# Zhengjun-Du/LC-CRF-SLAM

Hardware: NVIDIA B200
Metric: crf_problems_per_s (higher is better)
Workload: dtype f32

## Files before the change

### include/lccrf.h

```cpp
#ifndef LCCRF_H
#define LCCRF_H

#include <stdint.h>

#ifdef __cplusplus
extern "C" {
#endif

#define LCCRF_OK 0
#define LCCRF_ERR_ARG (-1)
#define LCCRF_ERR_CUDA (-2)
#define LCCRF_ERR_STATE (-3)
#define LCCRF_ERR_RANGE (-4)

#define LCCRF_MAX_D 7
#define LCCRF_MAX_L 64
#define LCCRF_MAX_K 8

typedef struct lccrf_ctx lccrf_ctx;
typedef struct lccrf_lattice lccrf_lattice;
typedef struct lccrf_crf lccrf_crf;
typedef struct lccrf_frames lccrf_frames;

const char *lccrf_version(void);
const char *lccrf_last_error(void);
int lccrf_device_count(void);
int lccrf_ctx_create(int device, lccrf_ctx **out);
void lccrf_ctx_destroy(lccrf_ctx *ctx);
int lccrf_ctx_set_stream(lccrf_ctx *ctx, void *cuda_stream);
int lccrf_ctx_sync(lccrf_ctx *ctx);
uint64_t lccrf_ctx_kernel_launches(const lccrf_ctx *ctx);
int lccrf_ctx_build_scratch_in_use(lccrf_ctx *ctx, long long *slots);
int lccrf_ctx_set_option(lccrf_ctx *ctx, const char *name, int value);
int lccrf_ctx_profile_report(lccrf_ctx *ctx, char *buf, int cap);

int lccrf_lattice_create(lccrf_ctx *ctx, const float *features, int d, int N, lccrf_lattice **out);
void lccrf_lattice_destroy(lccrf_lattice *lat);
int lccrf_lattice_sizes(const lccrf_lattice *lat, int *N, int *d, int *V);
int lccrf_lattice_export(const lccrf_lattice *lat, int *offset, float *bary, int *nbr);
int lccrf_lattice_filter(lccrf_lattice *lat, float *out, const float *in, int L);
int lccrf_lattice_filter_window(lccrf_lattice *lat, float *out, const float *in, int L, int in_offset, int out_offset,
                                int in_size, int out_size);

int lccrf_crf_create(lccrf_ctx *ctx, int N, int L, lccrf_crf **out);
void lccrf_crf_destroy(lccrf_crf *crf);
int lccrf_crf_set_unary(lccrf_crf *crf, const float *unary);
int lccrf_crf_set_unary_from_label(lccrf_crf *crf, const short *label, float u_energy,
                                   const float *n_energies, const float *p_energies);
int lccrf_crf_set_unary_entry(lccrf_crf *crf, int idx, int m, float value);
int lccrf_crf_add_potts(lccrf_crf *crf, const float *features, int d, float w);
int lccrf_crf_add_potts_image(lccrf_crf *crf, int W, int H, float w, float posdev, const void *img,
                              int img_is_u8, int F, float featuredev);
int lccrf_crf_start(lccrf_crf *crf);
int lccrf_crf_step(lccrf_crf *crf, float relax);
int lccrf_crf_inference(lccrf_crf *crf, int n_iterations, int with_map, float relax);
int lccrf_crf_build_map(lccrf_crf *crf);
const short *lccrf_crf_map(lccrf_crf *crf);
const float *lccrf_crf_prob(lccrf_crf *crf);
int lccrf_crf_potts_vertices(const lccrf_crf *crf, int k, int *V);
int lccrf_crf_num_potts(const lccrf_crf *crf);

int lccrf_crf_potts_apply(lccrf_crf *crf, int k, float *out, const float *in, float *tmp);
int lccrf_crf_step_init(lccrf_crf *crf, float *next);
int lccrf_crf_set_prob(lccrf_crf *crf, const float *prob);
int lccrf_exp_and_normalize(lccrf_ctx *ctx, float *out, const float *in, int N, int L, float scale,
                            float relax);

typedef struct lccrf_slam_params {
    float w1, w2;
    float u_alpha, stdev_alpha;
    float u_beta, stdev_beta;
    float u_gamma, stdev_gamma;
    float point3d_stdev, point2d_stdev;
    float u_depth, pth, confidence;
    int iters;
} lccrf_slam_params;

int lccrf_map_point_unary(lccrf_ctx *ctx, int N, const float *xyz, const int *obs_ptr, const int *obs_kf,
                          const float *obs_uv, int nKF, const float *kf_pose, const float *kf_intr,
                          const float *kf_bounds, float *observs, float *error, float *depth);
int lccrf_rough_classify(lccrf_ctx *ctx, int N, const float *observs, const float *error, const float *depth,
                         const double *p4, const lccrf_slam_params *prm, short *label);

int lccrf_epipolar_prior(lccrf_ctx *ctx, int M, const int *fid1, const float *pt1, const float *pt2,
                         const double *F9, float u_gamma, float stdev_gamma, int nFeat, double *dis_by_fid,
                         double *prob_by_fid, double *dis, double *prob);
int lccrf_bf_match(lccrf_ctx *ctx, int nq, const uint8_t *desc_q, int nt, const uint8_t *desc_t, double ratio,
                   int *match, int *knn, int *n_match);
int lccrf_bf_match_batch(lccrf_ctx *ctx, int B, const int *q_ptr, const uint8_t *desc_q, const int *t_ptr,
                         const uint8_t *desc_t, double ratio, int *match, int *knn, int *n_match);

int lccrf_frames_create(lccrf_ctx *ctx, int B, const int *prob_ptr, const lccrf_slam_params *prm,
                        const float *energies3, lccrf_frames **out);
void lccrf_frames_destroy(lccrf_frames *fr);
int lccrf_frames_set_inputs(lccrf_frames *fr, const float *observs, const float *error, const float *depth,
                            const float *kp2d);
int lccrf_frames_set_map_inputs(lccrf_frames *fr, const float *xyz, const int *obs_ptr, const int *obs_kf,
                                const float *obs_uv, int nKF, const float *kf_pose, const float *kf_intr,
                                const float *kf_bounds, const float *kp2d, const int *kf_ptr);
int lccrf_frames_run(lccrf_frames *fr);
int lccrf_frames_get_outputs(lccrf_frames *fr, short *map, float *prob);
int lccrf_frames_submit_map(lccrf_frames *fr, int slot, const float *xyz, const int *obs_ptr, const void *obs_kf,
                            int obs_kf_bytes, const float *obs_uv, int nKF, const float *kf_pose, const float *kf_intr,
                            const float *kf_bounds, const float *kp2d, const int *kf_ptr, short *map_out,
                            float *prob_out);
int lccrf_frames_set_keyframe_keypoints(lccrf_frames *fr, int kf_first, int kf_count, int stride, const float *kp_uv);
int lccrf_frames_set_map_inputs_indexed(lccrf_frames *fr, const float *xyz, const int *obs_ptr, const void *obs_ref,
                                        int index_bytes, int nKF, const float *kf_pose, const float *kf_intr,
                                        const float *kf_bounds, const float *kp2d, const int *kf_ptr);
int lccrf_frames_submit_map_indexed(lccrf_frames *fr, int slot, const float *xyz, const int *obs_ptr, const void *obs_ref,
                                    int index_bytes, int nKF, const float *kf_pose, const float *kf_intr,
                                    const float *kf_bounds, const float *kp2d, const int *kf_ptr, short *map_out,
                                    float *prob_out);
int lccrf_frames_submit(lccrf_frames *fr, int slot, const float *observs, const float *error, const float *depth,
                        const float *kp2d, short *map_out, float *prob_out);
int lccrf_frames_wait(lccrf_frames *fr, int slot);
int lccrf_frames_partition(lccrf_frames *fr, const int *fid, int *dyn_ptr, int *dyn_list, int *stat_ptr,
                           int *stat_list);
int lccrf_frames_get_debug(lccrf_frames *fr, short *init_label, float *observs, float *error, float *depth,
                           int *V);
int lccrf_frames_debug_counters(lccrf_frames *fr, int k, int *out8);
int lccrf_frames_algorithmic_bytes(lccrf_frames *fr, double *total, double *per_iteration, double *unary);

typedef struct lccrf_images lccrf_images;
typedef struct lccrf_image_kernel {
    int F;
    float w, posdev, featuredev;
} lccrf_image_kernel;
int  lccrf_images_create(lccrf_ctx *ctx, int B, const int *W, const int *H, int C, int L, int K,
                         const lccrf_image_kernel *kernels, lccrf_images **out);
void lccrf_images_destroy(lccrf_images *im);
int  lccrf_images_set_inputs(lccrf_images *im, const void *img, int img_is_u8, const float *unary);
int  lccrf_images_set_inputs_from_label(lccrf_images *im, const void *img, int img_is_u8, const short *label,
                                        float u_energy, const float *n_energies, const float *p_energies);
int  lccrf_images_run(lccrf_images *im, int n_iterations, float relax);
int  lccrf_images_get_outputs(lccrf_images *im, short *map, float *prob);
int  lccrf_images_vertices(lccrf_images *im, int *V);

typedef struct lccrf_map lccrf_map;
typedef struct lccrf_map_delta {
    int kf_first, kf_count;
    const float *kf_pose, *kf_intr, *kf_bounds, *kf_keypoints;
    int n_pose;
    const int *pose_kf;
    const float *pose;
    int n_xyz;
    const int *xyz_id;
    const float *xyz;
    int n_erase;
    const int *erase_pt, *erase_kf;
    int n_bad;
    const int *bad_pt;
    int n_add;
    const int *add_pt, *add_kf, *add_fid;
    int n_erase_seg;
    const int *erase_seg_ptr;
    int n_add_seg;
    const int *add_seg_ptr;
} lccrf_map_delta;
int lccrf_map_create(lccrf_ctx *ctx, int kp_stride, lccrf_map **out);
void lccrf_map_destroy(lccrf_map *map);
int lccrf_map_apply(lccrf_map *map, const lccrf_map_delta *delta);
int lccrf_map_set_observations(lccrf_map *map, int pt_first, int count, const int *obs_ptr, const int *obs_ref);
int lccrf_map_reserve_observations(lccrf_map *map, long long entries);
int lccrf_map_sizes(lccrf_map *map, int *n_kf, int *n_points, long long *n_obs, long long *pool_used, long long *pool_cap);
int lccrf_map_export(lccrf_map *map, int n, const int *point_id, int *obs_ptr, int *obs_kf, float *obs_uv, long long cap,
                     float *xyz);

int lccrf_frames_set_visible(lccrf_frames *fr, lccrf_map *map, const lccrf_map_delta *delta, const int *point_id,
                             const float *kp2d, const int *kf_ptr);
int lccrf_frames_submit_visible(lccrf_frames *fr, int slot, lccrf_map *map, const lccrf_map_delta *delta,
                                const int *point_id, const float *kp2d, const int *kf_ptr, short *map_out, float *prob_out);
int lccrf_frames_set_prior(lccrf_frames *fr, int slot, const double *p4, const unsigned char *has_prior);
int lccrf_frames_set_partition_outputs(lccrf_frames *fr, int slot, const int *fid, int *dyn_ptr, int *dyn_list, int *stat_ptr,
                                       int *stat_list);

typedef struct lccrf_snapshot_writer lccrf_snapshot_writer;
typedef struct lccrf_snapshot_reader lccrf_snapshot_reader;
typedef struct lccrf_snapshot_info {
    int N, nKF;
    long long nnz;
    long long frame_id;
    double timestamp;
    int stored_kf_bytes;
} lccrf_snapshot_info;
int lccrf_snapshot_writer_open(const char *path, int append, lccrf_snapshot_writer **out);
int lccrf_snapshot_write_frame(lccrf_snapshot_writer *w, long long frame_id, double timestamp, int N, const float *xyz,
                               const int *obs_ptr, const int *obs_kf, const float *obs_uv, int nKF, const float *kf_pose,
                               const float *kf_intr, const float *kf_bounds, const float *kp2d, const int *fid);
int lccrf_snapshot_writer_close(lccrf_snapshot_writer *w);
int lccrf_snapshot_reader_open(const char *path, lccrf_snapshot_reader **out);
void lccrf_snapshot_reader_close(lccrf_snapshot_reader *r);
int lccrf_snapshot_num_frames(const lccrf_snapshot_reader *r);
int lccrf_snapshot_truncated(const lccrf_snapshot_reader *r);
int lccrf_snapshot_frame_info(const lccrf_snapshot_reader *r, int i, lccrf_snapshot_info *info);
int lccrf_snapshot_read_frame(lccrf_snapshot_reader *r, int i, float *xyz, int *obs_ptr, void *obs_kf, int obs_kf_bytes,
                              float *obs_uv, float *kf_pose, float *kf_intr, float *kf_bounds, float *kp2d, int *fid);

#ifdef __cplusplus
}
#endif
#endif
```

### lc-crf-slam_b200/__init__.py

```python
from __future__ import annotations

import ctypes as C
import os
import subprocess
import weakref

import numpy as np

HERE = os.path.dirname(os.path.abspath(__file__))
LIB_PATH = os.path.join(HERE, "liblccrf.so")
INCLUDE_DIR = os.path.join(os.path.dirname(HERE), "include")
DENSECRF_INCLUDE_DIR = os.path.join(HERE, "densecrf")

from . import synth


def build(verbose: bool = False) -> str:
    subprocess.run(["make", "-C", os.path.join(HERE, "csrc"), "-j8"], check=True,
                   stdout=None if verbose else subprocess.DEVNULL)
    return LIB_PATH


class LccrfError(RuntimeError):
    pass


class SlamParams(C.Structure):
    _fields_ = [(n, C.c_float) for n in (
        "w1", "w2", "u_alpha", "stdev_alpha", "u_beta", "stdev_beta", "u_gamma", "stdev_gamma",
        "point3d_stdev", "point2d_stdev", "u_depth", "pth", "confidence")] + [("iters", C.c_int)]

    @classmethod
    def make(cls, **kw) -> "SlamParams":
        p = cls()
        d = dict(synth.SLAM_PARAMS)
        d.update(kw)
        for k, v in d.items():
            setattr(p, k, v)
        return p


class ImageKernel(C.Structure):
    _fields_ = [("F", C.c_int), ("w", C.c_float), ("posdev", C.c_float), ("featuredev", C.c_float)]


_fp = C.POINTER(C.c_float)
_ip = C.POINTER(C.c_int)
_sp = C.POINTER(C.c_short)
_vp = C.c_void_p
_byref = C.byref

SYMBOLS = {
    "lccrf_version": (C.c_char_p, []),
    "lccrf_last_error": (C.c_char_p, []),
    "lccrf_device_count": (C.c_int, []),
    "lccrf_ctx_create": (C.c_int, [C.c_int, C.POINTER(_vp)]),
    "lccrf_ctx_destroy": (None, [_vp]),
    "lccrf_ctx_set_stream": (C.c_int, [_vp, _vp]),
    "lccrf_ctx_sync": (C.c_int, [_vp]),
    "lccrf_ctx_kernel_launches": (C.c_uint64, [_vp]),
    "lccrf_ctx_build_scratch_in_use": (C.c_int, [_vp, _vp]),
    "lccrf_ctx_set_option": (C.c_int, [_vp, C.c_char_p, C.c_int]),
    "lccrf_ctx_profile_report": (C.c_int, [_vp, C.c_char_p, C.c_int]),
    "lccrf_lattice_create": (C.c_int, [_vp, _vp, C.c_int, C.c_int, C.POINTER(_vp)]),
    "lccrf_lattice_destroy": (None, [_vp]),
    "lccrf_lattice_sizes": (C.c_int, [_vp, _ip, _ip, _ip]),
    "lccrf_lattice_export": (C.c_int, [_vp, _vp, _vp, _vp]),
    "lccrf_lattice_filter": (C.c_int, [_vp, _vp, _vp, C.c_int]),
    "lccrf_lattice_filter_window": (C.c_int, [_vp, _vp, _vp, C.c_int, C.c_int, C.c_int, C.c_int, C.c_int]),
    "lccrf_crf_create": (C.c_int, [_vp, C.c_int, C.c_int, C.POINTER(_vp)]),
    "lccrf_crf_destroy": (None, [_vp]),
    "lccrf_crf_set_unary": (C.c_int, [_vp, _vp]),
    "lccrf_crf_set_unary_from_label": (C.c_int, [_vp, _vp, C.c_float, _vp, _vp]),
    "lccrf_crf_set_unary_entry": (C.c_int, [_vp, C.c_int, C.c_int, C.c_float]),
    "lccrf_crf_add_potts": (C.c_int, [_vp, _vp, C.c_int, C.c_float]),
    "lccrf_crf_add_potts_image": (C.c_int, [_vp, C.c_int, C.c_int, C.c_float, C.c_float, _vp, C.c_int, C.c_int, C.c_float]),
    "lccrf_crf_start": (C.c_int, [_vp]),
    "lccrf_crf_step": (C.c_int, [_vp, C.c_float]),
    "lccrf_crf_inference": (C.c_int, [_vp, C.c_int, C.c_int, C.c_float]),
    "lccrf_crf_build_map": (C.c_int, [_vp]),
    "lccrf_crf_map": (_sp, [_vp]),
    "lccrf_crf_prob": (_fp, [_vp]),
    "lccrf_crf_potts_vertices": (C.c_int, [_vp, C.c_int, _ip]),
    "lccrf_crf_num_potts": (C.c_int, [_vp]),
    "lccrf_crf_step_init": (C.c_int, [_vp, _vp]),
    "lccrf_crf_set_prob": (C.c_int, [_vp, _vp]),
    "lccrf_crf_potts_apply": (C.c_int, [_vp, C.c_int, _vp, _vp, _vp]),
    "lccrf_exp_and_normalize": (C.c_int, [_vp, _vp, _vp, C.c_int, C.c_int, C.c_float, C.c_float]),
    "lccrf_map_point_unary": (C.c_int, [_vp, C.c_int, _vp, _vp, _vp, _vp, C.c_int, _vp, _vp, _vp, _vp, _vp, _vp]),
    "lccrf_rough_classify": (C.c_int, [_vp, C.c_int, _vp, _vp, _vp, _vp, C.POINTER(SlamParams), _vp]),
    "lccrf_epipolar_prior": (C.c_int, [_vp, C.c_int, _vp, _vp, _vp, _vp, C.c_float, C.c_float, C.c_int, _vp, _vp, _vp, _vp]),
    "lccrf_bf_match": (C.c_int, [_vp, C.c_int, _vp, C.c_int, _vp, C.c_double, _vp, _vp, _ip]),
    "lccrf_bf_match_batch": (C.c_int, [_vp, C.c_int, _vp, _vp, _vp, _vp, C.c_double, _vp, _vp, _ip]),
    "lccrf_frames_create": (C.c_int, [_vp, C.c_int, _vp, C.POINTER(SlamParams), _vp, C.POINTER(_vp)]),
    "lccrf_frames_destroy": (None, [_vp]),
    "lccrf_frames_set_inputs": (C.c_int, [_vp, _vp, _vp, _vp, _vp]),
    "lccrf_frames_set_map_inputs": (C.c_int, [_vp, _vp, _vp, _vp, _vp, C.c_int, _vp, _vp, _vp, _vp, _vp]),
    "lccrf_frames_run": (C.c_int, [_vp]),
    "lccrf_frames_get_outputs": (C.c_int, [_vp, _vp, _vp]),
    "lccrf_frames_submit_map": (C.c_int, [_vp, C.c_int, _vp, _vp, _vp, C.c_int, _vp, C.c_int, _vp, _vp, _vp, _vp, _vp, _vp, _vp]),
    "lccrf_frames_set_keyframe_keypoints": (C.c_int, [_vp, C.c_int, C.c_int, C.c_int, _vp]),
    "lccrf_frames_set_map_inputs_indexed": (C.c_int, [_vp, _vp, _vp, _vp, C.c_int, C.c_int, _vp, _vp, _vp, _vp, _vp]),
    "lccrf_frames_submit_map_indexed": (C.c_int, [_vp, C.c_int, _vp, _vp, _vp, C.c_int, C.c_int, _vp, _vp, _vp, _vp, _vp, _vp, _vp]),
    "lccrf_frames_submit": (C.c_int, [_vp, C.c_int, _vp, _vp, _vp, _vp, _vp, _vp]),
    "lccrf_frames_wait": (C.c_int, [_vp, C.c_int]),
    "lccrf_frames_partition": (C.c_int, [_vp, _vp, _vp, _vp, _vp, _vp]),
    "lccrf_frames_get_debug": (C.c_int, [_vp, _vp, _vp, _vp, _vp, _vp]),
    "lccrf_frames_debug_counters": (C.c_int, [_vp, C.c_int, _vp]),
    "lccrf_frames_algorithmic_bytes": (C.c_int, [_vp, C.POINTER(C.c_double), C.POINTER(C.c_double), C.POINTER(C.c_double)]),
    "lccrf_images_create": (C.c_int, [_vp, C.c_int, _vp, _vp, C.c_int, C.c_int, C.c_int, C.POINTER(ImageKernel), C.POINTER(_vp)]),
    "lccrf_images_destroy": (None, [_vp]),
    "lccrf_images_set_inputs": (C.c_int, [_vp, _vp, C.c_int, _vp]),
    "lccrf_images_set_inputs_from_label": (C.c_int, [_vp, _vp, C.c_int, _vp, C.c_float, _vp, _vp]),
    "lccrf_images_run": (C.c_int, [_vp, C.c_int, C.c_float]),
    "lccrf_images_get_outputs": (C.c_int, [_vp, _vp, _vp]),
    "lccrf_images_vertices": (C.c_int, [_vp, _vp]),
    "lccrf_map_create": (C.c_int, [_vp, C.c_int, C.POINTER(_vp)]),
    "lccrf_map_destroy": (None, [_vp]),
    "lccrf_map_apply": (C.c_int, [_vp, _vp]),
    "lccrf_map_set_observations": (C.c_int, [_vp, C.c_int, C.c_int, _vp, _vp]),
    "lccrf_map_reserve_observations": (C.c_int, [_vp, C.c_longlong]),
    "lccrf_map_sizes": (C.c_int, [_vp, _ip, _ip, C.POINTER(C.c_longlong), C.POINTER(C.c_longlong), C.POINTER(C.c_longlong)]),
    "lccrf_map_export": (C.c_int, [_vp, C.c_int, _vp, _vp, _vp, _vp, C.c_longlong, _vp]),
    "lccrf_frames_set_visible": (C.c_int, [_vp, _vp, _vp, _vp, _vp, _vp]),
    "lccrf_frames_submit_visible": (C.c_int, [_vp, C.c_int, _vp, _vp, _vp, _vp, _vp, _vp, _vp]),
    "lccrf_frames_set_prior": (C.c_int, [_vp, C.c_int, _vp, _vp]),
    "lccrf_frames_set_partition_outputs": (C.c_int, [_vp, C.c_int, _vp, _vp, _vp, _vp, _vp]),
    "lccrf_snapshot_writer_open": (C.c_int, [C.c_char_p, C.c_int, C.POINTER(_vp)]),
    "lccrf_snapshot_write_frame": (C.c_int, [_vp, C.c_longlong, C.c_double, C.c_int, _vp, _vp, _vp, _vp, C.c_int, _vp, _vp, _vp, _vp, _vp]),
    "lccrf_snapshot_writer_close": (C.c_int, [_vp]),
    "lccrf_snapshot_reader_open": (C.c_int, [C.c_char_p, C.POINTER(_vp)]),
    "lccrf_snapshot_reader_close": (None, [_vp]),
    "lccrf_snapshot_num_frames": (C.c_int, [_vp]),
    "lccrf_snapshot_truncated": (C.c_int, [_vp]),
    "lccrf_snapshot_frame_info": (C.c_int, [_vp, C.c_int, _vp]),
    "lccrf_snapshot_read_frame": (C.c_int, [_vp, C.c_int, _vp, _vp, _vp, C.c_int, _vp, _vp, _vp, _vp, _vp, _vp]),
}

_lib = None


def load_library() -> C.CDLL:
    global _lib
    if _lib is not None:
        return _lib
    if not os.path.exists(LIB_PATH):
        raise LccrfError(f"{LIB_PATH} is missing: run __graft_entry__.build() (there is no CPU fallback)")
    lib = C.CDLL(LIB_PATH)
    for name, (res, args) in SYMBOLS.items():
        fn = getattr(lib, name)
        fn.restype = res
        fn.argtypes = args
    _lib = lib
    return lib


def _ptr(a):
    return None if a is None else a.ctypes.data


def _arr(a, dtype):
    return None if a is None else np.ascontiguousarray(a, dtype=dtype)


_libm = None


def _logf(x) -> np.float32:
    global _libm
    if _libm is None:
        _libm = C.CDLL("libm.so.6")
        _libm.logf.restype = C.c_float
        _libm.logf.argtypes = [C.c_float]
    return np.float32(_libm.logf(C.c_float(float(x))))


def label_energies(L: int, conf: float) -> np.ndarray:
    f = np.float32
    return np.array([-_logf(f(1.0) / f(L)), -_logf((f(1.0) - f(conf)) / f(L - 1)), -_logf(f(conf))], dtype=np.float32)


class Context:

    def __init__(self, device: int = 0, stream: int | None = None):
        self.lib = load_library()
        h = _vp()
        self._check(self.lib.lccrf_ctx_create(device, C.byref(h)))
        self.h = h
        self.device = device
        self._children = weakref.WeakSet()
        if stream is not None:
            self._check(self.lib.lccrf_ctx_set_stream(self.h, _vp(stream)))

    def _check(self, rc: int):
        if rc != 0:
            raise LccrfError(f"liblccrf error {rc}: {self.lib.lccrf_last_error().decode()}")

    def close(self):
        if getattr(self, "h", None):
            for child in list(getattr(self, "_children", ())):
                try:
                    child.close()
                except Exception:
                    pass
            self.lib.lccrf_ctx_destroy(self.h)
            self.h = None

    def __del__(self):
        try:
            self.close()
        except Exception:
            pass

    def sync(self):
        self._check(self.lib.lccrf_ctx_sync(self.h))

    def set_option(self, name: str, value: int):
        self._check(self.lib.lccrf_ctx_set_option(self.h, name.encode(), value))

    def profile_report(self) -> dict:
        buf = C.create_string_buffer(1 << 16)
        n = self.lib.lccrf_ctx_profile_report(self.h, buf, len(buf))
        if n < 0:
            self._check(n)
        out = {}
        for line in buf.value.decode().splitlines():
            name, cnt, ms = line.split()
            out[name] = (int(cnt), float(ms))
        return out

    @property
    def kernel_launches(self) -> int:
        return int(self.lib.lccrf_ctx_kernel_launches(self.h))

    def build_scratch_in_use(self) -> int:
        n = C.c_longlong(0)
        self._check(self.lib.lccrf_ctx_build_scratch_in_use(self.h, C.byref(n)))
        return n.value

    def exp_and_normalize(self, x, scale: float, relax: float = 1.0, prev=None) -> np.ndarray:
        x = _arr(x, np.float32)
        N, L = x.shape
        out = _arr(prev, np.float32).copy() if prev is not None else np.zeros_like(x)
        self._check(self.lib.lccrf_exp_and_normalize(self.h, _ptr(out), _ptr(x), N, L, scale, relax))
        return out

    def map_point_unary(self, snap):
        N = snap.n
        ob, er, de = (np.empty(N, dtype=np.float32) for _ in range(3))
        self._check(self.lib.lccrf_map_point_unary(
            self.h, N, _ptr(snap.xyz), _ptr(snap.obs_ptr), _ptr(snap.obs_kf), _ptr(snap.obs_uv),
            snap.kf_pose.shape[0], _ptr(snap.kf_pose), _ptr(snap.kf_intr), _ptr(snap.kf_bounds),
            _ptr(ob), _ptr(er), _ptr(de)))
        return ob, er, de

    def rough_classify(self, observs, error, depth, prm: SlamParams, p4=None) -> np.ndarray:
        observs, error, depth = (_arr(a, np.float32) for a in (observs, error, depth))
        p4 = _arr(p4, np.float64)
        lab = np.empty(observs.size, dtype=np.int16)
        self._check(self.lib.lccrf_rough_classify(self.h, observs.size, _ptr(observs), _ptr(error), _ptr(depth),
                                                  _ptr(p4), C.byref(prm), _ptr(lab)))
        return lab


    def epipolar_prior(self, fid1, pt1, pt2, F, u_gamma, stdev_gamma, n_feat=0):
        pt1, pt2 = _arr(pt1, np.float32), _arr(pt2, np.float32)
        M = pt1.shape[0]
        fid = _arr(fid1, np.int32) if fid1 is not None else None
        F9 = np.ascontiguousarray(F, dtype=np.float64).reshape(9)
        dis, prob = np.empty(M, np.float64), np.empty(M, np.float64)
        dbf, pbf = np.empty(n_feat, np.float64), np.empty(n_feat, np.float64)
        self._check(self.lib.lccrf_epipolar_prior(self.h, M, _ptr(fid), _ptr(pt1), _ptr(pt2), _ptr(F9), u_gamma, stdev_gamma,
                                                  n_feat, _ptr(dbf) if n_feat and fid is not None else None,
                                                  _ptr(pbf) if n_feat and fid is not None else None, _ptr(dis), _ptr(prob)))
        return dis, prob, dbf, pbf

    def bf_match(self, desc_q, desc_t, ratio=0.6, want_knn=True):
        dq = np.ascontiguousarray(desc_q, dtype=np.uint8).reshape(-1, 32)
        dt = np.ascontiguousarray(desc_t, dtype=np.uint8).reshape(-1, 32)
        match = np.empty(dq.shape[0], np.int32)
        knn = np.empty((dq.shape[0], 4), np.int32) if want_knn else None
        n = C.c_int(0)
        self._check(self.lib.lccrf_bf_match(self.h, dq.shape[0], _ptr(dq), dt.shape[0], _ptr(dt), ratio, _ptr(match),
                                            _ptr(knn), C.byref(n)))
        return match, knn, n.value

    def bf_match_batch(self, q_ptr, desc_q, t_ptr, desc_t, ratio=0.6, want_knn=False):
        q_ptr, t_ptr = _arr(q_ptr, np.int32), _arr(t_ptr, np.int32)
        dq = np.ascontiguousarray(desc_q, dtype=np.uint8).reshape(-1, 32)
        dt = np.ascontiguousarray(desc_t, dtype=np.uint8).reshape(-1, 32)
        match = np.empty(dq.shape[0], np.int32)
        knn = np.empty((dq.shape[0], 4), np.int32) if want_knn else None
        n = C.c_int(0)
        self._check(self.lib.lccrf_bf_match_batch(self.h, q_ptr.size - 1, _ptr(q_ptr), _ptr(dq), _ptr(t_ptr), _ptr(dt), ratio,
                                                  _ptr(match), _ptr(knn), C.byref(n)))
        return match, knn, n.value


class Lattice:

    def __init__(self, ctx: Context, features):
        self.ctx = ctx
        f = _arr(features, np.float32)
        self.N, self.d = f.shape
        h = _vp()
        ctx._check(ctx.lib.lccrf_lattice_create(ctx.h, _ptr(f), self.d, self.N, C.byref(h)))
        self.h = h
        ctx._children.add(self)
        v = C.c_int()
        ctx._check(ctx.lib.lccrf_lattice_sizes(self.h, None, None, C.byref(v)))
        self.V = v.value

    def export(self):
        D = self.d + 1
        off = np.empty((self.N, D), dtype=np.int32)
        bary = np.empty((self.N, D), dtype=np.float32)
        nbr = np.empty((D, self.V, 2), dtype=np.int32)
        self.ctx._check(self.ctx.lib.lccrf_lattice_export(self.h, _ptr(off), _ptr(bary), _ptr(nbr)))
        return off, bary, nbr

    def filter(self, x) -> np.ndarray:
        x = _arr(x, np.float32)
        L = x.size // self.N if self.N else 1
        out = np.empty_like(x)
        self.ctx._check(self.ctx.lib.lccrf_lattice_filter(self.h, _ptr(out), _ptr(x), L))
        return out

    def filter_window(self, x, L, in_offset=0, out_offset=0, in_size=-1, out_size=-1) -> np.ndarray:
        x = _arr(x, np.float32)
        n_out = self.N - out_offset if out_size == -1 else out_size
        out = np.empty((max(n_out, 0), L), dtype=np.float32)
        self.ctx._check(self.ctx.lib.lccrf_lattice_filter_window(self.h, _ptr(out), _ptr(x), L, in_offset, out_offset, in_size, out_size))
        return out

    def close(self):
        if getattr(self, "h", None):
            self.ctx.lib.lccrf_lattice_destroy(self.h)
            self.h = None

    def __del__(self):
        try:
            self.close()
        except Exception:
            pass


class DenseCRF:

    def __init__(self, ctx: Context, N: int, L: int):
        self.ctx, self.N, self.L = ctx, N, L
        h = _vp()
        ctx._check(ctx.lib.lccrf_crf_create(ctx.h, N, L, C.byref(h)))
        self.h = h
        ctx._children.add(self)

    def setUnaryEnergy(self, unary):
        u = _arr(unary, np.float32)
        self.ctx._check(self.ctx.lib.lccrf_crf_set_unary(self.h, _ptr(u)))

    def setUnaryEnergyFromLabel(self, label, confidence=0.5, energies=None):
        lab = _arr(label, np.int16)
        if energies is None:
            energies = label_energies(self.L, confidence)
        n_en = np.full(self.L, energies[1], dtype=np.float32)
        p_en = np.full(self.L, energies[2], dtype=np.float32)
        self.ctx._check(self.ctx.lib.lccrf_crf_set_unary_from_label(self.h, _ptr(lab), float(energies[0]), _ptr(n_en), _ptr(p_en)))

    def SetUnaryEnergtForPositiveNode(self, idx, m, value):
        self.ctx._check(self.ctx.lib.lccrf_crf_set_unary_entry(self.h, idx, m, value))

    def addPairwiseEnergy(self, features, w: float):
        f = _arr(features, np.float32)
        self.ctx._check(self.ctx.lib.lccrf_crf_add_potts(self.h, _ptr(f), f.shape[1], w))

    def addPairwiseFromImage(self, W, H, w, posdev, img=None, featuredev=0.0):
        if img is None:
            self.ctx._check(self.ctx.lib.lccrf_crf_add_potts_image(self.h, W, H, w, posdev, None, 0, 2, 0.0))
        else:
            is_u8 = img.dtype == np.uint8
            a = np.ascontiguousarray(img) if is_u8 else _arr(img, np.float32)
            F = 2 + a.size // (W * H)
            self.ctx._check(self.ctx.lib.lccrf_crf_add_potts_image(self.h, W, H, w, posdev, _ptr(a), int(is_u8), F, featuredev))

    def potts_vertices(self, k: int) -> int:
        v = C.c_int()
        self.ctx._check(self.ctx.lib.lccrf_crf_potts_vertices(self.h, k, C.byref(v)))
        return v.value

    def potts_apply(self, k, out, inp):
        out = _arr(out, np.float32).copy()
        inp = _arr(inp, np.float32)
        tmp = np.empty_like(out)
        self.ctx._check(self.ctx.lib.lccrf_crf_potts_apply(self.h, k, _ptr(out), _ptr(inp), _ptr(tmp)))
        return out, tmp

    def startInference(self):
        self.ctx._check(self.ctx.lib.lccrf_crf_start(self.h))

    def stepInference(self, relax=1.0):
        self.ctx._check(self.ctx.lib.lccrf_crf_step(self.h, relax))

    def inference(self, n_iterations, with_map=False, relax=1.0):
        self.ctx._check(self.ctx.lib.lccrf_crf_inference(self.h, n_iterations, int(with_map), relax))

    def buildMap(self):
        self.ctx._check(self.ctx.lib.lccrf_crf_build_map(self.h))

    def getMap(self):
        p = self.ctx.lib.lccrf_crf_map(self.h)
        if not p:
            return None
        return np.ctypeslib.as_array(p, shape=(max(self.N, 1),))[:self.N].copy()

    def getProbability(self):
        p = self.ctx.lib.lccrf_crf_prob(self.h)
        if not p:
            return None
        return np.ctypeslib.as_array(p, shape=(max(self.N, 1) * self.L,))[:self.N * self.L].copy().reshape(self.N, self.L)

    def close(self):
        if getattr(self, "h", None):
            self.ctx.lib.lccrf_crf_destroy(self.h)
            self.h = None

    def __del__(self):
        try:
            self.close()
        except Exception:
            pass


class MapDelta(C.Structure):
    _fields_ = [("kf_first", C.c_int), ("kf_count", C.c_int), ("kf_pose", _vp), ("kf_intr", _vp), ("kf_bounds", _vp),
                ("kf_keypoints", _vp), ("n_pose", C.c_int), ("pose_kf", _vp), ("pose", _vp), ("n_xyz", C.c_int),
                ("xyz_id", _vp), ("xyz", _vp), ("n_erase", C.c_int), ("erase_pt", _vp), ("erase_kf", _vp),
                ("n_bad", C.c_int), ("bad_pt", _vp), ("n_add", C.c_int), ("add_pt", _vp), ("add_kf", _vp), ("add_fid", _vp),
                ("n_erase_seg", C.c_int), ("erase_seg_ptr", _vp), ("n_add_seg", C.c_int), ("add_seg_ptr", _vp)]

    @classmethod
    def make(cls, kf_first=0, kf_pose=None, kf_intr=None, kf_bounds=None, kf_keypoints=None, pose_kf=None, pose=None,
             xyz_id=None, xyz=None, erase_pt=None, erase_kf=None, bad_pt=None, add_pt=None, add_kf=None, add_fid=None,
             erase_seg_ptr=None, add_seg_ptr=None, pin=None) -> "MapDelta":
        d = cls()
        keep = []

        def f32(a):
            if a is None:
                return None
            a = np.ascontiguousarray(a, dtype=np.float32)
            a = pin(a) if pin else a
            keep.append(a)
            return a

        def i32(a):
            if a is None:
                return None
            a = np.ascontiguousarray(a, dtype=np.int32)
            a = pin(a) if pin else a
            keep.append(a)
            return a

        kf_pose, kf_intr, kf_bounds, kf_keypoints, pose, xyz = (f32(a) for a in (kf_pose, kf_intr, kf_bounds, kf_keypoints, pose, xyz))
        pose_kf, xyz_id, erase_pt, erase_kf, bad_pt, add_pt, add_kf, add_fid = (
            i32(a) for a in (pose_kf, xyz_id, erase_pt, erase_kf, bad_pt, add_pt, add_kf, add_fid))
        d.kf_first = int(kf_first)
        d.kf_count = 0 if kf_pose is None else int(kf_pose.size // 12)
        d.kf_pose, d.kf_intr, d.kf_bounds, d.kf_keypoints = _ptr(kf_pose), _ptr(kf_intr), _ptr(kf_bounds), _ptr(kf_keypoints)
        d.n_pose = 0 if pose is None else int(pose.size // 12)
        d.pose_kf, d.pose = _ptr(pose_kf), _ptr(pose)
        d.n_xyz = 0 if xyz is None else int(xyz.size // 3)
        d.xyz_id, d.xyz = _ptr(xyz_id), _ptr(xyz)
        d.n_erase = 0 if erase_pt is None else int(erase_pt.size)
        d.erase_pt, d.erase_kf = _ptr(erase_pt), _ptr(erase_kf)
        d.n_bad = 0 if bad_pt is None else int(bad_pt.size)
        d.bad_pt = _ptr(bad_pt)
        d.n_add = 0 if add_pt is None else int(add_pt.size)
        d.add_pt, d.add_kf, d.add_fid = _ptr(add_pt), _ptr(add_kf), _ptr(add_fid)
        d._seg = [None if a is None else np.ascontiguousarray(a, dtype=np.int32) for a in (erase_seg_ptr, add_seg_ptr)]
        d.n_erase_seg = 0 if d._seg[0] is None else int(d._seg[0].size - 1)
        d.n_add_seg = 0 if d._seg[1] is None else int(d._seg[1].size - 1)
        d.erase_seg_ptr, d.add_seg_ptr = _ptr(d._seg[0]), _ptr(d._seg[1])
        if pose_kf is not None and pose_kf.size != d.n_pose or xyz_id is not None and xyz_id.size != d.n_xyz:
            raise LccrfError("MapDelta: id arrays must match their value arrays")
        if d.n_erase and (erase_kf is None or erase_kf.size != d.n_erase):
            raise LccrfError("MapDelta: erase_pt / erase_kf sizes differ")
        if d.n_add and (add_kf is None or add_fid is None or add_kf.size != d.n_add or add_fid.size != d.n_add):
            raise LccrfError("MapDelta: add_pt / add_kf / add_fid sizes differ")
        d._keep = keep
        return d

    @property
    def nbytes(self) -> int:
        return int(sum(a.nbytes for a in self._keep))


class Map:

    def __init__(self, ctx: Context, kp_stride: int):
        self.ctx, self.kp_stride = ctx, int(kp_stride)
        h = _vp()
        ctx._check(ctx.lib.lccrf_map_create(ctx.h, self.kp_stride, C.byref(h)))
        self.h = h
        ctx._children.add(self)

    def apply(self, delta: MapDelta = None, **kw):
        d = delta if delta is not None else MapDelta.make(**kw)
        self.ctx._check(self.ctx.lib.lccrf_map_apply(self.h, C.byref(d)))

    def set_observations(self, obs_ptr, obs_ref, pt_first=0):
        obs_ptr = _arr(obs_ptr, np.int32)
        obs_ref = _arr(obs_ref, np.int32)
        assert obs_ref.ndim == 2 and obs_ref.shape[1] == 2
        self.ctx._check(self.ctx.lib.lccrf_map_set_observations(self.h, int(pt_first), int(obs_ptr.size - 1), _ptr(obs_ptr), _ptr(obs_ref)))

    def reserve_observations(self, entries: int):
        self.ctx._check(self.ctx.lib.lccrf_map_reserve_observations(self.h, int(entries)))

    def sizes(self) -> dict:
        nk, npnt = C.c_int(), C.c_int()
        no, pu, pc = C.c_longlong(), C.c_longlong(), C.c_longlong()
        self.ctx._check(self.ctx.lib.lccrf_map_sizes(self.h, C.byref(nk), C.byref(npnt), C.byref(no), C.byref(pu), C.byref(pc)))
        return dict(n_kf=nk.value, n_points=npnt.value, n_obs=no.value, pool_used=pu.value, pool_cap=pc.value)

    def export(self, point_id):
        ids = _arr(point_id, np.int32)
        n = int(ids.size)
        ptr = np.zeros(n + 1, np.int32)
        self.ctx._check(self.ctx.lib.lccrf_map_export(self.h, n, _ptr(ids), _ptr(ptr), None, None, 0, None))
        nnz = int(ptr[-1])
        kf, uv, xyz = np.empty(nnz, np.int32), np.empty((nnz, 2), np.float32), np.empty((n, 3), np.float32)
        self.ctx._check(self.ctx.lib.lccrf_map_export(self.h, n, _ptr(ids), _ptr(ptr), _ptr(kf), _ptr(uv), nnz, _ptr(xyz)))
        return ptr, kf, uv, xyz

    def close(self):
        if getattr(self, "h", None):
            self.ctx.lib.lccrf_map_destroy(self.h)
            self.h = None

    def __del__(self):
        try:
            self.close()
        except Exception:
            pass


class Frames:

    def __init__(self, ctx: Context, n_points, prm: SlamParams | None = None, energies=None):
        self.ctx = ctx
        self.prm = prm or SlamParams.make()
        n_points = np.asarray(n_points, dtype=np.int64)
        self.B = int(n_points.size)
        self.prob_ptr = np.zeros(self.B + 1, dtype=np.int32)
        np.cumsum(n_points, out=self.prob_ptr[1:])
        self.NT = int(self.prob_ptr[-1])
        self.energies = label_energies(2, self.prm.confidence) if energies is None else _arr(energies, np.float32)
        h = _vp()
        ctx._check(ctx.lib.lccrf_frames_create(ctx.h, self.B, _ptr(self.prob_ptr), C.byref(self.prm), _ptr(self.energies), C.byref(h)))
        self.h = h
        ctx._children.add(self)

    def set_inputs(self, observs, error, depth, kp2d):
        a = [_arr(x, np.float32) for x in (observs, error, depth, kp2d)]
        self._keep = a
        self.ctx._check(self.ctx.lib.lccrf_frames_set_inputs(self.h, *[_ptr(x) for x in a]))

    def set_map_inputs(self, xyz, obs_ptr, obs_kf, obs_uv, kf_pose, kf_intr, kf_bounds, kp2d, kf_ptr=None):
        xyz, obs_uv, kf_pose, kf_intr, kf_bounds, kp2d = (_arr(x, np.float32) for x in (xyz, obs_uv, kf_pose, kf_intr, kf_bounds, kp2d))
        obs_ptr, obs_kf, kf_ptr = _arr(obs_ptr, np.int32), _arr(obs_kf, np.int32), _arr(kf_ptr, np.int32)
        self._keep = [xyz, obs_ptr, obs_kf, obs_uv, kf_pose, kf_intr, kf_bounds, kp2d, kf_ptr]
        self.ctx._check(self.ctx.lib.lccrf_frames_set_map_inputs(
            self.h, _ptr(xyz), _ptr(obs_ptr), _ptr(obs_kf), _ptr(obs_uv), kf_pose.shape[0], _ptr(kf_pose),
            _ptr(kf_intr), _ptr(kf_bounds), _ptr(kp2d), _ptr(kf_ptr)))

    def run(self):
        self.ctx._check(self.ctx.lib.lccrf_frames_run(self.h))

    def get_outputs(self, map_out=None, prob_out=None, want_prob=True):
        mp = np.empty(self.NT, dtype=np.int16) if map_out is None else map_out
        pr = (np.empty((self.NT, 2), dtype=np.float32) if prob_out is None else prob_out) if want_prob else None
        self.ctx._check(self.ctx.lib.lccrf_frames_get_outputs(self.h, _ptr(mp), _ptr(pr)))
        return mp, pr

    def submit_map(self, slot, xyz, obs_ptr, obs_kf, obs_uv, kf_pose, kf_intr, kf_bounds, kp2d, kf_ptr, map_out, prob_out):
        kb = obs_kf.dtype.itemsize
        assert obs_kf.dtype in (np.int32, np.uint16)
        self.ctx._check(self.ctx.lib.lccrf_frames_submit_map(
            self.h, slot, _ptr(xyz), _ptr(obs_ptr), _ptr(obs_kf), kb, _ptr(obs_uv), kf_pose.shape[0], _ptr(kf_pose),
            _ptr(kf_intr), _ptr(kf_bounds), _ptr(kp2d), _ptr(kf_ptr), _ptr(map_out), _ptr(prob_out)))

    def set_keyframe_keypoints(self, kp_table, kf_first=0):
        kp_table = _arr(kp_table, np.float32)
        assert kp_table.ndim == 3 and kp_table.shape[2] == 2
        self.ctx._check(self.ctx.lib.lccrf_frames_set_keyframe_keypoints(self.h, kf_first, kp_table.shape[0], kp_table.shape[1], _ptr(kp_table)))

    def set_map_inputs_indexed(self, xyz, obs_ptr, obs_ref, kf_pose, kf_intr, kf_bounds, kp2d, kf_ptr=None):
        xyz, kf_pose, kf_intr, kf_bounds, kp2d = (_arr(x, np.float32) for x in (xyz, kf_pose, kf_intr, kf_bounds, kp2d))
        obs_ptr, kf_ptr = _arr(obs_ptr, np.int32), _arr(kf_ptr, np.int32)
        obs_ref = np.ascontiguousarray(obs_ref)
        assert obs_ref.dtype in (np.int32, np.uint16) and obs_ref.ndim == 2 and obs_ref.shape[1] == 2
        self._keep = [xyz, obs_ptr, obs_ref, kf_pose, kf_intr, kf_bounds, kp2d, kf_ptr]
        self.ctx._check(self.ctx.lib.lccrf_frames_set_map_inputs_indexed(
            self.h, _ptr(xyz), _ptr(obs_ptr), _ptr(obs_ref), obs_ref.dtype.itemsize, kf_pose.shape[0], _ptr(kf_pose),
            _ptr(kf_intr), _ptr(kf_bounds), _ptr(kp2d), _ptr(kf_ptr)))

    def submit_map_indexed(self, slot, xyz, obs_ptr, obs_ref, kf_pose, kf_intr, kf_bounds, kp2d, kf_ptr, map_out, prob_out):
        assert obs_ref.dtype in (np.int32, np.uint16) and obs_ref.ndim == 2 and obs_ref.shape[1] == 2
        self.ctx._check(self.ctx.lib.lccrf_frames_submit_map_indexed(
            self.h, slot, _ptr(xyz), _ptr(obs_ptr), _ptr(obs_ref), obs_ref.dtype.itemsize, kf_pose.shape[0], _ptr(kf_pose),
            _ptr(kf_intr), _ptr(kf_bounds), _ptr(kp2d), _ptr(kf_ptr), _ptr(map_out), _ptr(prob_out)))

    def submit(self, slot, observs, error, depth, kp2d, map_out, prob_out):
        self.ctx._check(self.ctx.lib.lccrf_frames_submit(self.h, slot, _ptr(observs), _ptr(error), _ptr(depth), _ptr(kp2d),
                                                          _ptr(map_out), _ptr(prob_out)))

    def wait(self, slot):
        self.ctx._check(self.ctx.lib.lccrf_frames_wait(self.h, slot))

    def set_visible(self, mp: "Map", point_id, kp2d, delta: MapDelta = None, kf_ptr=None):
        ids, kp, kfp = _arr(point_id, np.int32), _arr(kp2d, np.float32), _arr(kf_ptr, np.int32)
        self.ctx._check(self.ctx.lib.lccrf_frames_set_visible(self.h, mp.h, C.byref(delta) if delta is not None else None,
                                                            _ptr(ids), _ptr(kp), _ptr(kfp)))

# ... 250 lines not shown
```

### lc-crf-slam_b200/csrc/api.cu

```cuda
#include <cstdio>
#include <cstring>
#include <string>
#include <vector>

#include "engine.cuh"

namespace lccrf {

static thread_local std::string g_err;
void set_error(const std::string &msg) { g_err = msg; }
int fail(int code, const std::string &msg) {
    g_err = msg;
    return code;
}

int dev_alloc(Ctx *ctx, void **p, size_t bytes, bool zero) {
    *p = nullptr;
    if (bytes == 0) bytes = 16;
    cudaError_t e = cudaMallocAsync(p, bytes, ctx->stream);
    if (e != cudaSuccess) return fail(LCCRF_ERR_CUDA, std::string("cudaMallocAsync: ") + cudaGetErrorString(e));
    if (zero) {
        e = cudaMemsetAsync(*p, 0, bytes, ctx->stream);
        if (e != cudaSuccess) return fail(LCCRF_ERR_CUDA, std::string("cudaMemsetAsync: ") + cudaGetErrorString(e));
    }
// ... 139 lines not shown
int graph_run(Ctx *ctx, GraphReplay &g, const std::function<int()> &enqueue) {
    if (!ctx->opt_graphs || ctx->opt_profile) return enqueue();
    if (g.exec && g.gen != ctx->scratch_gen) graph_drop(g);
    if (!g.exec && g.same_shape_runs == 0) {
        g.same_shape_runs = 1;
        return enqueue();
    }
    if (!g.exec) {
        const uint64_t l0 = ctx->launches;
        LCCRF_TRY(enqueue());
        LCCRF_CUDA(cudaStreamSynchronize(ctx->stream));
        const uint64_t per_run = ctx->launches - l0;
        cudaGraph_t cg = nullptr;
        LCCRF_CUDA(cudaStreamBeginCapture(ctx->stream, cudaStreamCaptureModeThreadLocal));
        int rc = enqueue();
        cudaError_t e = cudaStreamEndCapture(ctx->stream, &cg);
        ctx->launches -= per_run;
        if (rc != LCCRF_OK) {
            if (cg) cudaGraphDestroy(cg);
            return rc;
        }
        if (e != cudaSuccess) return fail(LCCRF_ERR_CUDA, std::string("graph capture: ") + cudaGetErrorString(e));
        e = cudaGraphInstantiate(&g.exec, cg, 0);
        cudaGraphDestroy(cg);
        if (e != cudaSuccess) return fail(LCCRF_ERR_CUDA, std::string("graph instantiate: ") + cudaGetErrorString(e));
        g.launches = per_run;
        g.gen = ctx->scratch_gen;
        return LCCRF_OK;
    }
    LCCRF_CUDA(cudaGraphLaunch(g.exec, ctx->stream));
    ctx->launches += g.launches;
    return LCCRF_OK;
}

}

using namespace lccrf;

struct lccrf_lattice {
    Ctx *ctx = nullptr;
    Batch b;
    LatticeSet *ls = nullptr;
    int V = 0;
    float *io = nullptr;
    size_t io_bytes = 0;
};

struct lccrf_crf {
    Ctx *ctx = nullptr;
    Batch b;
    bool started = false;
    float *h_prob = nullptr;
    short *h_map = nullptr;
    bool prob_fresh = false, map_fresh = false, map_built = false;
    float *d_energies = nullptr;
};

extern "C" {

const char *lccrf_version(void) { return "lccrf-b200 0.1 (sm_100a)"; }
const char *lccrf_last_error(void) { return g_err.c_str(); }

int lccrf_device_count(void) {
    int n = 0;
    if (cudaGetDeviceCount(&n) != cudaSuccess) return 0;
    return n;
}

int lccrf_ctx_create(int device, lccrf_ctx **out) {
    if (!out) return fail(LCCRF_ERR_ARG, "out is NULL");
    *out = nullptr;
    int n = 0;
    cudaError_t e = cudaGetDeviceCount(&n);
    if (e != cudaSuccess || n == 0)
        return fail(LCCRF_ERR_CUDA, std::string("no CUDA device available (there is no CPU fallback): ") +
                                        (e != cudaSuccess ? cudaGetErrorString(e) : "device count is 0"));
    if (device < 0 || device >= n) return fail(LCCRF_ERR_ARG, "device index out of range");
    LCCRF_CUDA(cudaSetDevice(device));
    cudaDeviceProp prop;
    LCCRF_CUDA(cudaGetDeviceProperties(&prop, device));
    if (prop.major != 10)
        return fail(LCCRF_ERR_CUDA, std::string("liblccrf is built for sm_100a only; device is ") + prop.name);
    auto *h = new lccrf_ctx();
    h->c.device = device;
    cudaError_t es = cudaStreamCreateWithFlags(&h->c.stream, cudaStreamNonBlocking);
    if (es != cudaSuccess) {
        delete h;
        return fail(LCCRF_ERR_CUDA, std::string("cudaStreamCreate: ") + cudaGetErrorString(es));
    }
    h->c.own_stream = true;
    if (cudaStreamCreateWithFlags(&h->c.aux_stream, cudaStreamNonBlocking) != cudaSuccess ||
        cudaEventCreateWithFlags(&h->c.ev_fork, cudaEventDisableTiming) != cudaSuccess ||
        cudaEventCreateWithFlags(&h->c.ev_join, cudaEventDisableTiming) != cudaSuccess) {
        delete h;
        return fail(LCCRF_ERR_CUDA, "aux stream / event creation failed");
    }
    for (int i = 0; i < 2; i++)
        if (cudaStreamCreateWithFlags(&h->c.sub_stream[i], cudaStreamNonBlocking) != cudaSuccess ||
            cudaEventCreateWithFlags(&h->c.ev_sub_fork[i], cudaEventDisableTiming) != cudaSuccess ||
            cudaEventCreateWithFlags(&h->c.ev_sub_join[i], cudaEventDisableTiming) != cudaSuccess) {
            delete h;
            return fail(LCCRF_ERR_CUDA, "sub stream / event creation failed");
        }
    cudaMemPool_t pool;
    if (cudaDeviceGetDefaultMemPool(&pool, device) == cudaSuccess) {
        uint64_t thr = UINT64_MAX;
        cudaMemPoolSetAttribute(pool, cudaMemPoolAttrReleaseThreshold, &thr);
    }
    if (cudaMalloc((void **)&h->c.d_status, sizeof(int)) != cudaSuccess ||
        cudaMemset(h->c.d_status, 0, sizeof(int)) != cudaSuccess ||
        cudaHostAlloc((void **)&h->c.h_status, sizeof(int), cudaHostAllocDefault) != cudaSuccess) {
        delete h;
        return fail(LCCRF_ERR_CUDA, "status word allocation failed");
    }
    *out = h;
    return LCCRF_OK;
}

void lccrf_ctx_destroy(lccrf_ctx *h) {
    if (!h) return;
    Ctx *c = &h->c;
    cudaSetDevice(c->device);
    cudaStreamSynchronize(c->stream);
    if (c->aux_stream) cudaStreamSynchronize(c->aux_stream);
    for (auto &bs : c->bs) {
        for (auto &s : bs.hash_keys) scratch_release(c, s, false);
        scratch_release(c, bs.hash_first, false);
        scratch_release(c, bs.hash_id, false);
        scratch_release(c, bs.ent_slot, false);
        scratch_release(c, bs.ids_status, false);
    }
    scratch_release(c, c->misc, false);
    scratch_release(c, c->feat, false);
    scratch_release(c, c->dev_io, false);
    scratch_release(c, c->pinned_in, true);
    scratch_release(c, c->pinned_out, true);
    cudaStreamSynchronize(c->stream);
    cudaFree(c->d_status);
    cudaFreeHost(c->h_status);
    if (c->copy_stream) cudaStreamDestroy(c->copy_stream);
    if (c->d2h_stream) cudaStreamDestroy(c->d2h_stream);
    if (c->aux_stream) cudaStreamDestroy(c->aux_stream);
    if (c->ev_fork) cudaEventDestroy(c->ev_fork);
    if (c->ev_join) cudaEventDestroy(c->ev_join);
    for (int i = 0; i < 2; i++) {
        if (c->sub_stream[i]) cudaStreamDestroy(c->sub_stream[i]);
        if (c->ev_sub_fork[i]) cudaEventDestroy(c->ev_sub_fork[i]);
        if (c->ev_sub_join[i]) cudaEventDestroy(c->ev_sub_join[i]);
    }
    if (c->own_stream) cudaStreamDestroy(c->stream);
    delete h;
}

int lccrf_ctx_set_stream(lccrf_ctx *h, void *cuda_stream) {
    if (!h) return fail(LCCRF_ERR_ARG, "ctx is NULL");
    Ctx *c = &h->c;
    LCCRF_CUDA(cudaSetDevice(c->device));
    LCCRF_CUDA(cudaStreamSynchronize(c->stream));
    if (c->own_stream) cudaStreamDestroy(c->stream);
    if (cuda_stream) {
        c->stream = (cudaStream_t)cuda_stream;
        c->own_stream = false;
    } else {
        LCCRF_CUDA(cudaStreamCreateWithFlags(&c->stream, cudaStreamNonBlocking));
        c->own_stream = true;
    }
    return LCCRF_OK;
}

int lccrf_ctx_sync(lccrf_ctx *h) {
    if (!h) return fail(LCCRF_ERR_ARG, "ctx is NULL");
    LCCRF_CUDA(cudaStreamSynchronize(h->c.stream));
    return LCCRF_OK;
}

uint64_t lccrf_ctx_kernel_launches(const lccrf_ctx *h) { return h ? h->c.launches : 0; }

int lccrf_ctx_build_scratch_in_use(lccrf_ctx *h, long long *slots) {
    if (!h || !slots) return fail(LCCRF_ERR_ARG, "NULL argument");
    return build_scratch_in_use(&h->c, slots);
}

int lccrf_ctx_set_option(lccrf_ctx *h, const char *name, int value) {
    if (!h || !name) return fail(LCCRF_ERR_ARG, "NULL argument");
    Ctx &c = h->c;
    const struct {
        const char *name;
        int *opt;
    } sequence[] = {{"fused", &c.opt_fused}, {"ordered_splat", &c.opt_ordered_splat}, {"bulk_blur", &c.opt_bulk_blur},
                    {"concurrent", &c.opt_concurrent}, {"split_splat", &c.opt_split_splat}};
    for (const auto &s : sequence)
        if (!strcmp(name, s.name)) {
            if (*s.opt != (value ? 1 : 0)) c.scratch_gen++;
            *s.opt = value ? 1 : 0;
            return LCCRF_OK;
        }
    if (!strcmp(name, "graphs")) c.opt_graphs = value;
    else if (!strcmp(name, "profile")) c.opt_profile = value;
    else if (!strcmp(name, "map_slack")) c.opt_map_slack = value < 0 ? 0 : value;
    else if (!strcmp(name, "trace")) c.opt_trace = value;
    else return fail(LCCRF_ERR_ARG, std::string("unknown option ") + name);
    return LCCRF_OK;
}

int lccrf_ctx_profile_report(lccrf_ctx *h, char *buf, int cap) {
    if (!h || !buf || cap < 1) return fail(LCCRF_ERR_ARG, "NULL argument");
    Ctx *c = &h->c;
    LCCRF_CUDA(cudaSetDevice(c->device));
    LCCRF_CUDA(cudaStreamSynchronize(c->stream));
    std::vector<std::string> names;
    std::vector<double> ms;
    std::vector<long long> cnt;
    for (auto &r : c->prof) {
        float t = 0.f;
        cudaEventElapsedTime(&t, r.a, r.b);
        cudaEventDestroy(r.a);
        cudaEventDestroy(r.b);
        size_t k = 0;
        for (; k < names.size(); k++)
            if (names[k] == r.name) break;
        if (k == names.size()) {
            names.push_back(r.name);
            ms.push_back(0);
            cnt.push_back(0);
        }
        ms[k] += t;
        cnt[k]++;
    }
    c->prof.clear();
    std::string out;
    char line[256];
    for (size_t k = 0; k < names.size(); k++) {
        snprintf(line, sizeof(line), "%s %lld %.6f\n", names[k].c_str(), cnt[k], ms[k]);
        out += line;
    }
    strncpy(buf, out.c_str(), (size_t)cap - 1);
    buf[cap - 1] = 0;
    return (int)names.size();
}

int lccrf_lattice_create(lccrf_ctx *h, const float *features, int d, int N, lccrf_lattice **out) {
    if (!h || !out || (N > 0 && !features)) return fail(LCCRF_ERR_ARG, "NULL argument");
    if (N < 0) return fail(LCCRF_ERR_ARG, "N < 0");
    *out = nullptr;
    Ctx *ctx = &h->c;
    LCCRF_CUDA(cudaSetDevice(ctx->device));
    auto *lat = new lccrf_lattice();
    lat->ctx = ctx;
    int pp[2] = {0, N};
    int rc = batch_init(ctx, lat->b, 1, pp, 1, false);
    if (rc == LCCRF_OK) rc = lattice_set_create(ctx, lat->b, d, 1.0f, 0, &lat->ls);
    if (rc == LCCRF_OK) rc = ctx_scratch(ctx, ctx->feat, (size_t)(N > 0 ? N : 1) * d * sizeof(float));
    if (rc == LCCRF_OK && N > 0) {
        cudaError_t e = cudaMemcpyAsync(ctx->feat.p, features, (size_t)N * d * sizeof(float), cudaMemcpyHostToDevice, ctx->stream);
        if (e != cudaSuccess) rc = fail(LCCRF_ERR_CUDA, cudaGetErrorString(e));
    }
    if (rc == LCCRF_OK) rc = lattice_set_build(ctx, lat->b, lat->ls, (const float *)ctx->feat.p);
    if (rc == LCCRF_OK) {
        cudaError_t e = cudaMemcpyAsync(ctx->h_status, lat->ls->vbase + 1, sizeof(int), cudaMemcpyDeviceToHost, ctx->stream);
        if (e == cudaSuccess) e = cudaStreamSynchronize(ctx->stream);
        if (e != cudaSuccess) rc = fail(LCCRF_ERR_CUDA, cudaGetErrorString(e));
        else lat->V = *ctx->h_status;
    }
    if (rc == LCCRF_OK) rc = check_status(ctx);
    if (rc != LCCRF_OK) {
        lccrf_lattice_destroy(lat);
        return rc;
    }
    *out = lat;
    return LCCRF_OK;
}

void lccrf_lattice_destroy(lccrf_lattice *lat) {
    if (!lat) return;
    cudaSetDevice(lat->ctx->device);
    if (lat->ls) lattice_set_destroy(lat->ctx, lat->ls);
    lat->ls = nullptr;
    batch_release(lat->ctx, lat->b);
    dev_free(lat->ctx, lat->io);
    delete lat;
}

int lccrf_lattice_sizes(const lccrf_lattice *lat, int *N, int *d, int *V) {
    if (!lat) return fail(LCCRF_ERR_ARG, "lattice is NULL");
    if (N) *N = lat->b.NT;
    if (d) *d = lat->ls->d;
    if (V) *V = lat->V;
    return LCCRF_OK;
}

int lccrf_lattice_export(const lccrf_lattice *lat, int *offset, float *bary, int *nbr) {
    if (!lat) return fail(LCCRF_ERR_ARG, "lattice is NULL");
    Ctx *ctx = lat->ctx;
    LCCRF_CUDA(cudaSetDevice(ctx->device));
    const LatticeSet *ls = lat->ls;
    const size_t nent = (size_t)lat->b.NT * ls->D;
    if (offset && nent) LCCRF_CUDA(cudaMemcpyAsync(offset, ls->offset, nent * sizeof(int), cudaMemcpyDeviceToHost, ctx->stream));
    if (bary && nent) LCCRF_CUDA(cudaMemcpyAsync(bary, ls->bary, nent * sizeof(float), cudaMemcpyDeviceToHost, ctx->stream));
    if (nbr && lat->V > 0) {
        for (int j = 0; j < ls->D; j++)
            LCCRF_CUDA(cudaMemcpyAsync(nbr + 2 * (size_t)j * lat->V, ls->nbr + (size_t)j * ls->Vcap,
                                       (size_t)lat->V * sizeof(int2), cudaMemcpyDeviceToHost, ctx->stream));
    }
    LCCRF_CUDA(cudaStreamSynchronize(ctx->stream));
    return LCCRF_OK;
}

int lccrf_lattice_filter_window(lccrf_lattice *lat, float *out, const float *in, int L, int in_offset, int out_offset,
                                int in_size, int out_size) {
    if (!lat || !out || !in) return fail(LCCRF_ERR_ARG, "NULL argument");
    if (L < 1 || L > LCCRF_MAX_L) return fail(LCCRF_ERR_ARG, "L out of range");
    const int N = lat->b.NT;
    if (in_size == -1) in_size = N - in_offset;
    if (out_size == -1) out_size = N - out_offset;
    if (in_offset < 0 || out_offset < 0 || in_size < 0 || out_size < 0 || (long long)in_offset + in_size > N ||
        (long long)out_offset + out_size > N)
        return fail(LCCRF_ERR_ARG, "filter window outside [0, N)");
    Ctx *ctx = lat->ctx;
    LCCRF_CUDA(cudaSetDevice(ctx->device));
    const size_t n = (size_t)N * L;
    if (n == 0 || out_size == 0) return LCCRF_OK;
    LCCRF_TRY(lattice_set_ensure_L(ctx, lat->ls, L));
    if (lat->io_bytes < 2 * n * sizeof(float)) {
        dev_free(ctx, lat->io);
        lat->io = nullptr;
        lat->io_bytes = 0;
        LCCRF_TRY(dev_alloc(ctx, (void **)&lat->io, 2 * n * sizeof(float)));
        lat->io_bytes = 2 * n * sizeof(float);
    }
    float *d_in = lat->io, *d_out = lat->io + n;
    if (in_size != N) LCCRF_CUDA(cudaMemsetAsync(d_in, 0, n * sizeof(float), ctx->stream));
    if (in_size > 0)
        LCCRF_CUDA(cudaMemcpyAsync(d_in + (size_t)in_offset * L, in, (size_t)in_size * L * sizeof(float), cudaMemcpyHostToDevice, ctx->stream));
    LCCRF_TRY(filter_full(ctx, lat->b, lat->ls, d_out, d_in, L));
    LCCRF_CUDA(cudaMemcpyAsync(out, d_out + (size_t)out_offset * L, (size_t)out_size * L * sizeof(float), cudaMemcpyDeviceToHost, ctx->stream));
    LCCRF_CUDA(cudaStreamSynchronize(ctx->stream));
    return LCCRF_OK;
}

int lccrf_lattice_filter(lccrf_lattice *lat, float *out, const float *in, int L) {
    return lccrf_lattice_filter_window(lat, out, in, L, 0, 0, -1, -1);
}

int lccrf_crf_create(lccrf_ctx *h, int N, int L, lccrf_crf **out) {
    if (!h || !out) return fail(LCCRF_ERR_ARG, "NULL argument");
    if (N < 0 || L < 1 || L > LCCRF_MAX_L) return fail(LCCRF_ERR_ARG, "N or L out of range");
    *out = nullptr;
    Ctx *ctx = &h->c;
    LCCRF_CUDA(cudaSetDevice(ctx->device));
    auto *crf = new lccrf_crf();
    crf->ctx = ctx;
    int pp[2] = {0, N};
    int rc = batch_init(ctx, crf->b, 1, pp, L, true);
    if (rc == LCCRF_OK) rc = dev_alloc(ctx, (void **)&crf->d_energies, 2 * (size_t)L * sizeof(float));
    if (rc == LCCRF_OK) {
        const size_t n = (size_t)(N > 0 ? N : 1);
        if (cudaHostAlloc((void **)&crf->h_prob, n * L * sizeof(float), cudaHostAllocDefault) != cudaSuccess ||
            cudaHostAlloc((void **)&crf->h_map, n * sizeof(short), cudaHostAllocDefault) != cudaSuccess)
            rc = fail(LCCRF_ERR_CUDA, "pinned result buffers: cudaHostAlloc failed");
    }
    if (rc != LCCRF_OK) {
        lccrf_crf_destroy(crf);
        return rc;
    }
    *out = crf;
    return LCCRF_OK;
}

void lccrf_crf_destroy(lccrf_crf *crf) {
    if (!crf) return;
    cudaSetDevice(crf->ctx->device);
    cudaStreamSynchronize(crf->ctx->stream);
    batch_release(crf->ctx, crf->b);
    dev_free(crf->ctx, crf->d_energies);
    if (crf->h_prob) cudaFreeHost(crf->h_prob);
    if (crf->h_map) cudaFreeHost(crf->h_map);
    delete crf;
}

int lccrf_crf_set_unary(lccrf_crf *crf, const float *unary) {
    if (!crf || (!unary && crf->b.NT > 0)) return fail(LCCRF_ERR_ARG, "NULL argument");
    Ctx *ctx = crf->ctx;
    LCCRF_CUDA(cudaSetDevice(ctx->device));
    const size_t n = (size_t)crf->b.NT * crf->b.L;
    if (n) LCCRF_CUDA(cudaMemcpyAsync(crf->b.unary, unary, n * sizeof(float), cudaMemcpyHostToDevice, ctx->stream));
    LCCRF_CUDA(cudaStreamSynchronize(ctx->stream));
    return LCCRF_OK;
}

int lccrf_crf_set_unary_from_label(lccrf_crf *crf, const short *label, float u_energy, const float *n_energies,
                                   const float *p_energies) {
    if (!crf || !n_energies || !p_energies || (!label && crf->b.NT > 0)) return fail(LCCRF_ERR_ARG, "NULL argument");
    Ctx *ctx = crf->ctx;
    LCCRF_CUDA(cudaSetDevice(ctx->device));
    const int NT = crf->b.NT, L = crf->b.L;
    for (int i = 0; i < NT; i++)
        if (label[i] < -1 || label[i] >= L) return fail(LCCRF_ERR_ARG, "label outside [-1, L)");
    LCCRF_CUDA(cudaMemcpyAsync(crf->d_energies, n_energies, (size_t)L * sizeof(float), cudaMemcpyHostToDevice, ctx->stream));
    LCCRF_CUDA(cudaMemcpyAsync(crf->d_energies + L, p_energies, (size_t)L * sizeof(float), cudaMemcpyHostToDevice, ctx->stream));
    if (NT > 0) {
        LCCRF_TRY(ctx_scratch(ctx, ctx->dev_io, (size_t)NT * sizeof(short)));
        LCCRF_CUDA(cudaMemcpyAsync(ctx->dev_io.p, label, (size_t)NT * sizeof(short), cudaMemcpyHostToDevice, ctx->stream));
        LCCRF_TRY(mf_unary_from_label(ctx, crf->b.unary, (const short *)ctx->dev_io.p, NT, L, u_energy, crf->d_energies,
                                      crf->d_energies + L));
    }
    LCCRF_CUDA(cudaStreamSynchronize(ctx->stream));
    return LCCRF_OK;
}

int lccrf_crf_set_unary_entry(lccrf_crf *crf, int idx, int m, float value) {
    if (!crf) return fail(LCCRF_ERR_ARG, "crf is NULL");
    if (idx < 0 || idx >= crf->b.NT || m < 0 || m >= crf->b.L) return fail(LCCRF_ERR_ARG, "index out of range");
    Ctx *ctx = crf->ctx;
    LCCRF_CUDA(cudaSetDevice(ctx->device));
    LCCRF_CUDA(cudaMemcpyAsync(crf->b.unary + (size_t)idx * crf->b.L + m, &value, sizeof(float), cudaMemcpyHostToDevice, ctx->stream));
    LCCRF_CUDA(cudaStreamSynchronize(ctx->stream));
    return LCCRF_OK;
}

static int crf_add_lattice(lccrf_crf *crf, int d, float w, const float *feat_dev) {
    Ctx *ctx = crf->ctx;
    if ((int)crf->b.lat.size() >= LCCRF_MAX_K) return fail(LCCRF_ERR_ARG, "too many pairwise potentials");
    LatticeSet *ls = nullptr;
    LCCRF_TRY(lattice_set_create(ctx, crf->b, d, w, crf->b.L, &ls));
    int rc = lattice_set_build(ctx, crf->b, ls, feat_dev);
    if (rc == LCCRF_OK) rc = potts_norm(ctx, crf->b, ls);
    if (rc == LCCRF_OK) rc = check_status(ctx);
    if (rc != LCCRF_OK) {
        lattice_set_destroy(ctx, ls);
        return rc;
    }
    crf->b.lat.push_back(ls);
    return LCCRF_OK;
}

int lccrf_crf_add_potts(lccrf_crf *crf, const float *features, int d, float w) {
    if (!crf || (!features && crf->b.NT > 0)) return fail(LCCRF_ERR_ARG, "NULL argument");
    if (d < 1 || d > LCCRF_MAX_D) return fail(LCCRF_ERR_ARG, "feature dimension must be in [1, LCCRF_MAX_D]");
    Ctx *ctx = crf->ctx;
    LCCRF_CUDA(cudaSetDevice(ctx->device));
    const size_t n = (size_t)crf->b.NT * d;
    LCCRF_TRY(ctx_scratch(ctx, ctx->feat, (n ? n : 1) * sizeof(float)));
    if (n) LCCRF_CUDA(cudaMemcpyAsync(ctx->feat.p, features, n * sizeof(float), cudaMemcpyHostToDevice, ctx->stream));
    return crf_add_lattice(crf, d, w, (const float *)ctx->feat.p);
}

int lccrf_crf_add_potts_image(lccrf_crf *crf, int W, int H, float w, float posdev, const void *img, int img_is_u8,
                              int F, float featuredev) {
    if (!crf) return fail(LCCRF_ERR_ARG, "crf is NULL");
    if (W < 0 || H < 0 || (long long)W * H != crf->b.NT) return fail(LCCRF_ERR_ARG, "W*H must equal N");
    if (F < 2 || F > LCCRF_MAX_D) return fail(LCCRF_ERR_ARG, "F must be in [2, LCCRF_MAX_D]");
    if (F > 2 && !img && crf->b.NT > 0) return fail(LCCRF_ERR_ARG, "image features required when F > 2");
    Ctx *ctx = crf->ctx;
    LCCRF_CUDA(cudaSetDevice(ctx->device));
    const size_t npx = (size_t)crf->b.NT;
    LCCRF_TRY(ctx_scratch(ctx, ctx->feat, (npx ? npx : 1) * F * sizeof(float)));
    const void *img_dev = nullptr;
    if (F > 2 && npx) {
        const size_t ib = npx * (F - 2) * (img_is_u8 ? 1 : sizeof(float));
        LCCRF_TRY(ctx_scratch(ctx, ctx->dev_io, ib));
        LCCRF_CUDA(cudaMemcpyAsync(ctx->dev_io.p, img, ib, cudaMemcpyHostToDevice, ctx->stream));
        img_dev = ctx->dev_io.p;
    }
    LCCRF_TRY(feat_image(ctx, (float *)ctx->feat.p, W, H, F, posdev, img_dev, img_is_u8, featuredev));
    return crf_add_lattice(crf, F, w, (const float *)ctx->feat.p);
}

int lccrf_crf_start(lccrf_crf *crf) {
    if (!crf) return fail(LCCRF_ERR_ARG, "crf is NULL");
    LCCRF_CUDA(cudaSetDevice(crf->ctx->device));
    LCCRF_TRY(mf_start(crf->ctx, crf->b));
    crf->started = true;
    crf->prob_fresh = false;
    return LCCRF_OK;
}

int lccrf_crf_step(lccrf_crf *crf, float relax) {
    if (!crf) return fail(LCCRF_ERR_ARG, "crf is NULL");
    if (!crf->started) return fail(LCCRF_ERR_STATE, "stepInference before startInference");
    LCCRF_CUDA(cudaSetDevice(crf->ctx->device));
    LCCRF_TRY(mf_step(crf->ctx, crf->b, relax));
    crf->prob_fresh = false;
    return LCCRF_OK;
}

int lccrf_crf_build_map(lccrf_crf *crf) {
    if (!crf) return fail(LCCRF_ERR_ARG, "crf is NULL");
    LCCRF_CUDA(cudaSetDevice(crf->ctx->device));
    LCCRF_TRY(mf_build_map(crf->ctx, crf->b));
    crf->map_built = true;
    crf->map_fresh = false;
    return LCCRF_OK;
}

static int crf_fetch(lccrf_crf *crf) {
    Ctx *ctx = crf->ctx;
    const size_t n = (size_t)crf->b.NT;
    bool any = false;
    if (!crf->prob_fresh && n) {
        LCCRF_CUDA(cudaMemcpyAsync(crf->h_prob, crf->b.cur, n * crf->b.L * sizeof(float), cudaMemcpyDeviceToHost, ctx->stream));
        any = true;
    }
    if (crf->map_built && !crf->map_fresh && n) {
        LCCRF_CUDA(cudaMemcpyAsync(crf->h_map, crf->b.map, n * sizeof(short), cudaMemcpyDeviceToHost, ctx->stream));
        any = true;
    }
    if (any) LCCRF_CUDA(cudaStreamSynchronize(ctx->stream));
    crf->prob_fresh = true;
    if (crf->map_built) crf->map_fresh = true;
    return LCCRF_OK;
}

int lccrf_crf_inference(lccrf_crf *crf, int n_iterations, int with_map, float relax) {
    if (!crf) return fail(LCCRF_ERR_ARG, "crf is NULL");
    LCCRF_TRY(lccrf_crf_start(crf));
    for (int it = 0; it < n_iterations; it++) LCCRF_TRY(lccrf_crf_step(crf, relax));
    if (with_map) LCCRF_TRY(lccrf_crf_build_map(crf));
    return crf_fetch(crf);
}

const short *lccrf_crf_map(lccrf_crf *crf) {
    if (!crf || !crf->map_built) return nullptr;
    cudaSetDevice(crf->ctx->device);
    if (crf_fetch(crf) != LCCRF_OK) return nullptr;
    return crf->h_map;
}

const float *lccrf_crf_prob(lccrf_crf *crf) {
    if (!crf) return nullptr;
    cudaSetDevice(crf->ctx->device);
    if (!crf->started) {
        return crf->h_prob;
    }
    if (crf_fetch(crf) != LCCRF_OK) return nullptr;
    return crf->h_prob;
}

int lccrf_crf_potts_vertices(const lccrf_crf *crf, int k, int *V) {
    if (!crf || !V) return fail(LCCRF_ERR_ARG, "NULL argument");
    if (k < 0 || k >= (int)crf->b.lat.size()) return fail(LCCRF_ERR_ARG, "potential index out of range");
    Ctx *ctx = crf->ctx;
    LCCRF_CUDA(cudaSetDevice(ctx->device));
    LCCRF_CUDA(cudaMemcpyAsync(ctx->h_status, crf->b.lat[k]->vbase + 1, sizeof(int), cudaMemcpyDeviceToHost, ctx->stream));
    LCCRF_CUDA(cudaStreamSynchronize(ctx->stream));
    *V = *ctx->h_status;
    return LCCRF_OK;
}

int lccrf_crf_num_potts(const lccrf_crf *crf) { return crf ? (int)crf->b.lat.size() : 0; }

int lccrf_crf_step_init(lccrf_crf *crf, float *next) {
    if (!crf || !next) return fail(LCCRF_ERR_ARG, "NULL argument");
    Ctx *ctx = crf->ctx;
    LCCRF_CUDA(cudaSetDevice(ctx->device));
    const size_t n = (size_t)crf->b.NT * crf->b.L;
    if (!n) return LCCRF_OK;
    LCCRF_TRY(mf_negate(ctx, crf->b.next, crf->b.unary, (long long)n));
    LCCRF_CUDA(cudaMemcpyAsync(next, crf->b.next, n * sizeof(float), cudaMemcpyDeviceToHost, ctx->stream));
    LCCRF_CUDA(cudaStreamSynchronize(ctx->stream));
    return LCCRF_OK;
}

int lccrf_crf_set_prob(lccrf_crf *crf, const float *prob) {
    if (!crf || !prob) return fail(LCCRF_ERR_ARG, "NULL argument");
    Ctx *ctx = crf->ctx;
    LCCRF_CUDA(cudaSetDevice(ctx->device));
    const size_t n = (size_t)crf->b.NT * crf->b.L;
    if (n) LCCRF_CUDA(cudaMemcpyAsync(crf->b.cur, prob, n * sizeof(float), cudaMemcpyHostToDevice, ctx->stream));
    LCCRF_CUDA(cudaStreamSynchronize(ctx->stream));
    crf->started = true;
    crf->prob_fresh = false;
    return LCCRF_OK;
}

int lccrf_crf_potts_apply(lccrf_crf *crf, int k, float *out, const float *in, float *tmp) {
    if (!crf || !out || !in || !tmp) return fail(LCCRF_ERR_ARG, "NULL argument");
    if (k < 0 || k >= (int)crf->b.lat.size()) return fail(LCCRF_ERR_ARG, "potential index out of range");
    Ctx *ctx = crf->ctx;
    LCCRF_CUDA(cudaSetDevice(ctx->device));
    const size_t n = (size_t)crf->b.NT * crf->b.L;
    if (!n) return LCCRF_OK;
    LCCRF_TRY(ctx_scratch(ctx, ctx->dev_io, 3 * n * sizeof(float)));
    float *d_out = (float *)ctx->dev_io.p, *d_in = d_out + n, *d_tmp = d_in + n;
    LCCRF_CUDA(cudaMemcpyAsync(d_out, out, n * sizeof(float), cudaMemcpyHostToDevice, ctx->stream));
    LCCRF_CUDA(cudaMemcpyAsync(d_in, in, n * sizeof(float), cudaMemcpyHostToDevice, ctx->stream));
    LCCRF_TRY(mf_potts_apply(ctx, crf->b, crf->b.lat[k], d_out, d_in, d_tmp, crf->b.L));
    LCCRF_CUDA(cudaMemcpyAsync(out, d_out, n * sizeof(float), cudaMemcpyDeviceToHost, ctx->stream));
    LCCRF_CUDA(cudaMemcpyAsync(tmp, d_tmp, n * sizeof(float), cudaMemcpyDeviceToHost, ctx->stream));
    LCCRF_CUDA(cudaStreamSynchronize(ctx->stream));
    return LCCRF_OK;
}

int lccrf_exp_and_normalize(lccrf_ctx *h, float *out, const float *in, int N, int L, float scale, float relax) {
    if (!h || !out || !in) return fail(LCCRF_ERR_ARG, "NULL argument");
    if (N < 0 || L < 1 || L > LCCRF_MAX_L) return fail(LCCRF_ERR_ARG, "N or L out of range");
    Ctx *ctx = &h->c;
    LCCRF_CUDA(cudaSetDevice(ctx->device));
    const size_t n = (size_t)N * L;
    if (!n) return LCCRF_OK;
    LCCRF_TRY(ctx_scratch(ctx, ctx->dev_io, 2 * n * sizeof(float)));
    float *d_out = (float *)ctx->dev_io.p, *d_in = d_out + n;
    LCCRF_CUDA(cudaMemcpyAsync(d_in, in, n * sizeof(float), cudaMemcpyHostToDevice, ctx->stream));
    if (relax != 1.0f) LCCRF_CUDA(cudaMemcpyAsync(d_out, out, n * sizeof(float), cudaMemcpyHostToDevice, ctx->stream));
    LCCRF_TRY(mf_exp_and_normalize(ctx, d_out, d_in, N, L, scale, relax));
    LCCRF_CUDA(cudaMemcpyAsync(out, d_out, n * sizeof(float), cudaMemcpyDeviceToHost, ctx->stream));
    LCCRF_CUDA(cudaStreamSynchronize(ctx->stream));
// ... 357 lines not shown
```

### lc-crf-slam_b200/csrc/common.cuh

```cuda
#pragma once

#include <cuda_runtime.h>
#include <stdint.h>

#include <string>

#include "../../include/lccrf.h"

namespace lccrf {

void set_error(const std::string &msg);
int fail(int code, const std::string &msg);

#define LCCRF_CUDA(expr)                                                                          \
    do {                                                                                          \
        cudaError_t _e = (expr);                                                                  \
        if (_e != cudaSuccess)                                                                    \
            return ::lccrf::fail(LCCRF_ERR_CUDA, std::string(#expr) + ": " + cudaGetErrorString(_e)); \
    } while (0)

#define LCCRF_TRY(expr)            \
    do {                           \
        int _rc = (expr);          \
        if (_rc != LCCRF_OK) return _rc; \
    } while (0)

constexpr int kNumSMs = 148;
constexpr int kThreads = 256;

static inline int cdiv(long long a, long long b) { return (int)((a + b - 1) / b); }
static inline int persistent_grid(long long work_items, int threads = kThreads, int ctas_per_sm = 8) {
    long long need = (work_items + threads - 1) / threads;
    long long cap = (long long)kNumSMs * ctas_per_sm;
    if (need >= cap) return (int)cap;
    if (need > kNumSMs) need = (need + kNumSMs - 1) / kNumSMs * kNumSMs;
    return (int)(need < 1 ? 1 : need);
}

#ifdef __CUDACC__
__device__ __forceinline__ uint32_t mix64(uint64_t x) {
    x ^= x >> 33;
    x *= 0xff51afd7ed558ccdULL;
    x ^= x >> 33;
    x *= 0xc4ceb9fe1a85ec53ULL;
    x ^= x >> 33;
    return (uint32_t)x;
}

__device__ __forceinline__ int find_segment(const int *__restrict__ arr, int n, int x) {
    int lo = 0, hi = n;
    while (hi - lo > 1) {
        int mid = (lo + hi) >> 1;
        if (__ldg(arr + mid) <= x) lo = mid;
        else hi = mid;
    }
    return lo;
}
#endif

}
```

### lc-crf-slam_b200/csrc/csr.cu

```cuda
#include "engine.cuh"

namespace lccrf {

namespace {

constexpr int kFillThreads = 1024;
constexpr int kCursorSmemInts = 14336;

struct CsrParams {
    int G;
    int D;
    const int *chunk_prob;
    const int *chunk_s0;
    const int *chunk_s1;
    const long long *chunk_tbl;
    const int *prob_chunk0;
    const int *offset;
    const float *bary;
    const int *vbase;
    const int *vert_prob;
    int *tbl;
    int *row_len;
    int2 *ent;
};

__global__ void __launch_bounds__(kThreads) k_csr_zero(CsrParams p) {
    const int g = blockIdx.x;
    const int b = __ldg(p.chunk_prob + g);
    const int Vb = __ldg(p.vbase + b + 1) - __ldg(p.vbase + b);
    int *row = p.tbl + __ldg(p.chunk_tbl + g);
    for (int v = threadIdx.x; v < Vb; v += kThreads) row[v] = 0;
}

__global__ void __launch_bounds__(kFillThreads) k_csr_count(CsrParams p) {
    const int g = blockIdx.x;
    const int b = __ldg(p.chunk_prob + g);
    const int vb = __ldg(p.vbase + b);
    int *row = p.tbl + __ldg(p.chunk_tbl + g);
    const int s0 = __ldg(p.chunk_s0 + g), s1 = __ldg(p.chunk_s1 + g);
    const unsigned lane = threadIdx.x & 31;
    for (int base = s0; base < s1; base += 4 * kFillThreads) {
        int v[4];
#pragma unroll
        for (int j = 0; j < 4; j++) {
            const int s = base + j * kFillThreads + threadIdx.x;
            v[j] = s < s1 ? __ldg(p.offset + s) - vb : -1;
        }
#pragma unroll
        for (int j = 0; j < 4; j++) {
            const unsigned grp = __match_any_sync(0xffffffffu, v[j]);
            if (v[j] >= 0 && (__ffs(grp) - 1) == (int)lane) atomicAdd(row + v[j], __popc(grp));
        }
    }
}

__global__ void __launch_bounds__(kThreads) k_csr_prefix(CsrParams p, int B) {
    const int V = __ldg(p.vbase + B);
    for (int v = blockIdx.x * kThreads + threadIdx.x; v < V; v += gridDim.x * kThreads) {
        const int b = __ldg(p.vert_prob + v);
        const int lv = v - __ldg(p.vbase + b);
        const int g0 = __ldg(p.prob_chunk0 + b), g1 = __ldg(p.prob_chunk0 + b + 1);
        int run = 0;
        for (int g = g0; g < g1; g++) {
            int *c = p.tbl + __ldg(p.chunk_tbl + g) + lv;
            const int n = *c;
            *c = run;
            run += n;
        }
        p.row_len[v] = run;
    }
}

__global__ void __launch_bounds__(1024) k_scan_local(int *x, const int *n_ptr, int *blk_tot) {
    __shared__ int ws[32];
    const int n = __ldg(n_ptr);
    const int lane = threadIdx.x & 31, wid = threadIdx.x >> 5;
    for (int blk = blockIdx.x; blk * 1024 < n + 1; blk += gridDim.x) {
        const int idx = blk * 1024 + threadIdx.x;
        const int v = idx < n ? x[idx] : 0;
        int s = v;
#pragma unroll
        for (int o = 1; o < 32; o <<= 1) {
            int y = __shfl_up_sync(0xffffffffu, s, o);
            if (lane >= o) s += y;
        }
        if (lane == 31) ws[wid] = s;
        __syncthreads();
        if (wid == 0) {
            int t = ws[lane];
#pragma unroll
            for (int o = 1; o < 32; o <<= 1) {
                int y = __shfl_up_sync(0xffffffffu, t, o);
                if (lane >= o) t += y;
            }
            ws[lane] = t;
        }
        __syncthreads();
        const int excl = (wid ? ws[wid - 1] : 0) + s - v;
        if (idx <= n) x[idx] = excl;
        if (threadIdx.x == 1023) blk_tot[blk] = ws[31];
        __syncthreads();
    }
}

__global__ void __launch_bounds__(1024) k_scan_tot(int *blk_tot, const int *n_ptr) {
    __shared__ int ws[32];
    __shared__ int carry_s;
    const int nblk = (__ldg(n_ptr) + 1 + 1023) / 1024;
    if (threadIdx.x == 0) carry_s = 0;
    __syncthreads();
    const int lane = threadIdx.x & 31, wid = threadIdx.x >> 5;
    for (int start = 0; start < nblk; start += 1024) {
        const int idx = start + threadIdx.x;
        const int v = idx < nblk ? blk_tot[idx] : 0;
        int s = v;
#pragma unroll
        for (int o = 1; o < 32; o <<= 1) {
            int y = __shfl_up_sync(0xffffffffu, s, o);
            if (lane >= o) s += y;
        }
        if (lane == 31) ws[wid] = s;
        __syncthreads();
        if (wid == 0) {
            int t = ws[lane];
#pragma unroll
            for (int o = 1; o < 32; o <<= 1) {
                int y = __shfl_up_sync(0xffffffffu, t, o);
                if (lane >= o) t += y;
            }
            ws[lane] = t;
        }
        __syncthreads();
        const int carry = carry_s;
        if (idx < nblk) blk_tot[idx] = carry + (wid ? ws[wid - 1] : 0) + s - v;
        __syncthreads();
        if (threadIdx.x == 1023) carry_s = carry + ws[31];
        __syncthreads();
    }
}

__global__ void __launch_bounds__(1024) k_scan_add(int *x, const int *n_ptr, const int *blk_tot) {
    const int n = __ldg(n_ptr);
    for (int blk = blockIdx.x; blk * 1024 < n + 1; blk += gridDim.x) {
        const int idx = blk * 1024 + threadIdx.x;
        if (idx <= n) x[idx] += __ldg(blk_tot + blk);
    }
}

constexpr int kFillWarpsH = 8;
constexpr int kHierV = kCursorSmemInts / kFillWarpsH;

constexpr int kFillAhead = 4;

template <int MODE>
__device__ __forceinline__ void fill_walk(const CsrParams &p, int vb, int a, int z, int *cur_row, unsigned lane) {
    for (int base0 = a; base0 < z; base0 += 32 * kFillAhead) {
        int gv[kFillAhead], rp[kFillAhead];
        float w[kFillAhead];
#pragma unroll
        for (int g = 0; g < kFillAhead; g++) {
            const int s = base0 + 32 * g + (int)lane;
            gv[g] = s < z ? __ldg(p.offset + s) : -1;
            w[g] = s < z ? __ldg(p.bary + s) : 0.f;
        }
#pragma unroll
        for (int g = 0; g < kFillAhead; g++) rp[g] = gv[g] >= 0 ? __ldg(p.row_len + gv[g]) : 0;
#pragma unroll
        for (int g = 0; g < kFillAhead; g++) {
            if (base0 + 32 * g >= z) break;
            const int s = base0 + 32 * g + (int)lane;
            const int v = gv[g] >= 0 ? gv[g] - vb : -1;
            const unsigned grp = __match_any_sync(0xffffffffu, v);
            const int leader = __ffs(grp) - 1;
            const int rank = __popc(grp & ((1u << lane) - 1u));
            int cur = 0;
            if (v >= 0 && (int)lane == leader) {
                if (MODE == 2) {
                    cur = ((volatile int *)cur_row)[v];
                    ((volatile int *)cur_row)[v] = cur + __popc(grp);
                } else {
                    cur = cur_row[v];
                    cur_row[v] = cur + __popc(grp);
                }
            }
            __syncwarp();
            cur = __shfl_sync(0xffffffffu, cur, leader);
            if (v >= 0) p.ent[rp[g] + cur + rank] = make_int2(s / p.D, __float_as_int(w[g]));
        }
    }
}

__global__ void __launch_bounds__(kFillWarpsH * 32) k_csr_fill(CsrParams p) {
    extern __shared__ int s_cur[];
    const int g = blockIdx.x;
    const int b = __ldg(p.chunk_prob + g);
    const int vb = __ldg(p.vbase + b);
    const int Vb = __ldg(p.vbase + b + 1) - vb;
    int *row = p.tbl + __ldg(p.chunk_tbl + g);
    const int s0 = __ldg(p.chunk_s0 + g), s1 = __ldg(p.chunk_s1 + g);
    const unsigned lane = threadIdx.x & 31;
    const int wid = threadIdx.x >> 5;
    if (Vb <= kHierV) {
        const int sub = ((s1 - s0 + kFillWarpsH - 1) / kFillWarpsH + 31) & ~31;
        const int a = min(s0 + wid * sub, s1), z = min(a + sub, s1);
        int *mine = s_cur + wid * Vb;
        for (int v = threadIdx.x; v < kFillWarpsH * Vb; v += kFillWarpsH * 32) s_cur[v] = 0;
        __syncthreads();
        for (int base0 = a; base0 < z; base0 += 32 * kFillAhead) {
            int vv[kFillAhead];
#pragma unroll
            for (int g = 0; g < kFillAhead; g++) {
                const int s = base0 + 32 * g + (int)lane;
                vv[g] = s < z ? __ldg(p.offset + s) - vb : -1;
            }
#pragma unroll
            for (int g = 0; g < kFillAhead; g++) {
                const unsigned grp = __match_any_sync(0xffffffffu, vv[g]);
                if (vv[g] >= 0 && (__ffs(grp) - 1) == (int)lane) mine[vv[g]] += __popc(grp);
                __syncwarp();
            }
        }
        __syncthreads();
        for (int v = threadIdx.x; v < Vb; v += kFillWarpsH * 32) {
            int run = row[v];
#pragma unroll
            for (int w = 0; w < kFillWarpsH; w++) {
                const int n = s_cur[w * Vb + v];
                s_cur[w * Vb + v] = run;
                run += n;
            }
        }
        __syncthreads();
        fill_walk<0>(p, vb, a, z, mine, lane);
    } else if (wid == 0) {
        if (Vb <= kCursorSmemInts) {
            for (int v = (int)lane; v < Vb; v += 32) s_cur[v] = row[v];
            __syncwarp();
            fill_walk<1>(p, vb, s0, s1, s_cur, lane);
        } else {
            fill_walk<2>(p, vb, s0, s1, row, lane);
        }
    }
}

__global__ void __launch_bounds__(kThreads)
k_row_classify(const int *__restrict__ row_ptr, const int *__restrict__ vtotal, int *__restrict__ lng,
               int *__restrict__ counts, int *__restrict__ piece_list) {
    const int V = __ldg(vtotal);
    for (int v = blockIdx.x * kThreads + threadIdx.x; v < V; v += gridDim.x * kThreads) {
        const int start = __ldg(row_ptr + v);
        const int len = __ldg(row_ptr + v + 1) - start;
        if (len >= kLongRow) {
            lng[atomicAdd(counts, 1)] = v;
        } else {
            bool first = v == 0;
            if (!first) {
                const int pstart = __ldg(row_ptr + v - 1);
                first = (start - pstart >= kLongRow) || (start / kTileGranule != pstart / kTileGranule);
            }
            if (first) piece_list[atomicAdd(counts + 2, 1)] = v;
        }
    }
}

__global__ void __launch_bounds__(1024)
k_long_chunks(const int *__restrict__ row_ptr, const int *__restrict__ lng, int *__restrict__ counts,
              int *__restrict__ long_chunk0, int4 *__restrict__ chunk_desc) {
    __shared__ int ws[32];
    __shared__ int carry_s;
    const int n = counts[0];
    if (threadIdx.x == 0) carry_s = 0;
    __syncthreads();
    const int lane = threadIdx.x & 31, wid = threadIdx.x >> 5;
    for (int start = 0; start < n; start += 1024) {
        const int i = start + threadIdx.x;
        int nch = 0, rs = 0, re = 0;
        if (i < n) {
            const int v = lng[i];
            rs = __ldg(row_ptr + v);
            re = __ldg(row_ptr + v + 1);
            nch = (re - rs + kScanChunk - 1) / kScanChunk;
        }
        int x = nch;
#pragma unroll
        for (int o = 1; o < 32; o <<= 1) {
            int y = __shfl_up_sync(0xffffffffu, x, o);
            if (lane >= o) x += y;
        }
        if (lane == 31) ws[wid] = x;
        __syncthreads();
        if (wid == 0) {
            int t = ws[lane];
#pragma unroll
            for (int o = 1; o < 32; o <<= 1) {
                int y = __shfl_up_sync(0xffffffffu, t, o);
                if (lane >= o) t += y;
            }
            ws[lane] = t;
        }
        __syncthreads();
        const int carry = carry_s;
        const int base = carry + (wid ? ws[wid - 1] : 0) + x - nch;
        if (i < n) {
            long_chunk0[i] = base;
            for (int c = 0; c < nch; c++)
                chunk_desc[base + c] = make_int4(rs + c * kScanChunk, min(rs + (c + 1) * kScanChunk, re), base, i);
        }
        __syncthreads();
        if (threadIdx.x == 1023) carry_s = carry + ws[31];
        __syncthreads();
    }
    if (threadIdx.x == 0) {
        long_chunk0[n] = carry_s;
        counts[1] = carry_s;
    }
}

__global__ void __launch_bounds__(kThreads)
k_tile_rows(const int *__restrict__ row_ptr, const int *__restrict__ vtotal, int *__restrict__ tile_row0,
            int *__restrict__ tile_own, int n_tiles) {
    const int V = __ldg(vtotal);
    if (blockIdx.x == 0 && threadIdx.x == 0) tile_row0[n_tiles] = V - 1;
    for (int v = blockIdx.x * kThreads + threadIdx.x; v < V; v += gridDim.x * kThreads) {
        const int s = __ldg(row_ptr + v), e = __ldg(row_ptr + v + 1);
        for (int t = (s + kTreeTile - 1) / kTreeTile; t < n_tiles && t * kTreeTile < e; t++) tile_row0[t] = v;
        if (e - s < kLongRow && n_tiles > 0) {
            const int t = e > s ? s / kTreeTile : (s > 0 ? (s - 1) / kTreeTile : 0);
            tile_own[t < n_tiles ? t : n_tiles - 1] = 1;
        }
    }
}

}

int csr_create(Ctx *ctx, const Batch &b, LatticeSet *ls) {
    const int D = ls->D;
    std::vector<int> chunk_prob, chunk_s0, chunk_s1, prob_chunk0(b.B + 1);
    std::vector<long long> chunk_tbl;
    long long tbl = 0;
    for (long long min_cpts = kCsrChunkPoints;; min_cpts *= 2) {
        chunk_prob.clear();
        chunk_s0.clear();
        chunk_s1.clear();
        chunk_tbl.clear();
        tbl = 0;
        for (int i = 0; i < b.B; i++) {
            prob_chunk0[i] = (int)chunk_prob.size();
            const int p0 = b.h_prob_ptr[i], p1 = b.h_prob_ptr[i + 1];
            const long long stride = ((long long)(p1 - p0) + 1) * D;
            long long cpts = min_cpts;
            while (((long long)(p1 - p0) + cpts - 1) / cpts * stride > (1ll << 30)) cpts *= 2;
            for (long long c = p0; c < p1; c += cpts) {
                chunk_prob.push_back(i);
                chunk_s0.push_back((int)(c * D));
                chunk_s1.push_back((int)((c + cpts < p1 ? c + cpts : p1) * D));
                chunk_tbl.push_back(tbl);
                tbl += stride;
            }
        }
        if (tbl <= (1ll << 31) - 1 || min_cpts > b.maxN) break;
    }
    prob_chunk0[b.B] = (int)chunk_prob.size();
    ls->csr_chunks = (int)chunk_prob.size();
    if (tbl > (1ll << 31) - 1) return fail(LCCRF_ERR_ARG, "CSR count table would exceed 2^31 entries");
    const size_t G = (size_t)(ls->csr_chunks > 0 ? ls->csr_chunks : 1);
    int rc = LCCRF_OK;
    rc |= dev_alloc(ctx, (void **)&ls->chunk_prob, G * 4);
    rc |= dev_alloc(ctx, (void **)&ls->chunk_s0, G * 4);
    rc |= dev_alloc(ctx, (void **)&ls->chunk_s1, G * 4);
    rc |= dev_alloc(ctx, (void **)&ls->chunk_tbl, G * 8);
    rc |= dev_alloc(ctx, (void **)&ls->prob_chunk0, (size_t)(b.B + 1) * 4);
    rc |= dev_alloc(ctx, (void **)&ls->csr_tbl, (size_t)(tbl > 0 ? tbl : 1) * 4);
    rc |= dev_alloc(ctx, (void **)&ls->row_ptr, ((size_t)ls->Vcap + 2) * 4);
    rc |= dev_alloc(ctx, (void **)&ls->csr_ent, (size_t)(b.NT > 0 ? b.NT : 1) * D * sizeof(int2));
    rc |= dev_alloc(ctx, (void **)&ls->scan_tot, ((size_t)ls->Vcap / 1024 + 2) * 4);
    {
        const long long E = (long long)b.NT * D;
        ls->max_long = (int)(E / kLongRow);
        ls->max_chunks = (int)(E / kScanChunk) + ls->max_long;
    }
    rc |= dev_alloc(ctx, (void **)&ls->row_list_long, ((size_t)ls->max_long + 1) * 4);
    rc |= dev_alloc(ctx, (void **)&ls->long_chunk0, ((size_t)ls->max_long + 2) * 4);
    rc |= dev_alloc(ctx, (void **)&ls->chunk_desc, ((size_t)ls->max_chunks + 1) * 16);
    rc |= dev_alloc(ctx, (void **)&ls->row_counts, 16 * 4, true);
    ls->max_pieces = (int)(((long long)b.NT * D) / kTileGranule + ((long long)b.NT * D) / kLongRow + 2);
    rc |= dev_alloc(ctx, (void **)&ls->piece_list, (size_t)ls->max_pieces * 4);
    ls->n_tiles = (int)(((long long)b.NT * D + kTreeTile - 1) / kTreeTile);
    rc |= dev_alloc(ctx, (void **)&ls->tile_row0, ((size_t)ls->n_tiles + 1) * 4);
    rc |= dev_alloc(ctx, (void **)&ls->tile_own, ((size_t)ls->n_tiles + 1) * 4);
    rc |= dev_alloc(ctx, (void **)&ls->tile_info, ((size_t)ls->n_tiles + 1) * sizeof(int2));
    if (ls->Lmax > 0) rc |= dev_alloc(ctx, (void **)&ls->tile_part, ((size_t)ls->n_tiles + 1) * ls->Lmax * sizeof(float));
    if (rc != LCCRF_OK) return LCCRF_ERR_CUDA;
    cudaStream_t st = ctx->stream;
    if (ls->csr_chunks > 0) {
        LCCRF_CUDA(cudaMemcpyAsync(ls->chunk_prob, chunk_prob.data(), G * 4, cudaMemcpyHostToDevice, st));
        LCCRF_CUDA(cudaMemcpyAsync(ls->chunk_s0, chunk_s0.data(), G * 4, cudaMemcpyHostToDevice, st));
        LCCRF_CUDA(cudaMemcpyAsync(ls->chunk_s1, chunk_s1.data(), G * 4, cudaMemcpyHostToDevice, st));
        LCCRF_CUDA(cudaMemcpyAsync(ls->chunk_tbl, chunk_tbl.data(), G * 8, cudaMemcpyHostToDevice, st));
    }
    LCCRF_CUDA(cudaMemcpyAsync(ls->prob_chunk0, prob_chunk0.data(), (size_t)(b.B + 1) * 4, cudaMemcpyHostToDevice, st));
    LCCRF_CUDA(cudaStreamSynchronize(st));
    return LCCRF_OK;
}

void csr_destroy(Ctx *ctx, LatticeSet *ls) {
    dev_free(ctx, ls->chunk_prob);
    dev_free(ctx, ls->chunk_s0);
    dev_free(ctx, ls->chunk_s1);
    dev_free(ctx, ls->chunk_tbl);
    dev_free(ctx, ls->prob_chunk0);
    dev_free(ctx, ls->csr_tbl);
    dev_free(ctx, ls->row_ptr);
    dev_free(ctx, ls->csr_ent);
    dev_free(ctx, ls->scan_tot);
    dev_free(ctx, ls->row_list_long);
    dev_free(ctx, ls->long_chunk0);
    dev_free(ctx, ls->chunk_desc);
    dev_free(ctx, ls->chunk_sum);
    dev_free(ctx, ls->chunk_rec);
    dev_free(ctx, ls->row_counts);
    dev_free(ctx, ls->piece_list);
    dev_free(ctx, ls->tile_row0);
    dev_free(ctx, ls->tile_own);
    dev_free(ctx, ls->tile_info);
    dev_free(ctx, ls->tile_part);
}

int csr_build(Ctx *ctx, const Batch &b, LatticeSet *ls) {
    cudaStream_t st = ctx->stream;
    CsrParams p;
    p.G = ls->csr_chunks;
    p.D = ls->D;
    p.chunk_prob = ls->chunk_prob;
    p.chunk_s0 = ls->chunk_s0;
    p.chunk_s1 = ls->chunk_s1;
    p.chunk_tbl = ls->chunk_tbl;
    p.prob_chunk0 = ls->prob_chunk0;
    p.offset = ls->offset;
    p.bary = ls->bary;
    p.vbase = ls->vbase;
    p.vert_prob = ls->vert_prob;
    p.tbl = ls->csr_tbl;
    p.row_len = ls->row_ptr;
    p.ent = ls->csr_ent;
    const int *vt = ls->vbase + ls->B;
    if (p.G > 0) {
        { LCCRF_KERNEL(ctx, "k_csr_zero"); k_csr_zero<<<p.G, kThreads, 0, st>>>(p); }
        { LCCRF_KERNEL(ctx, "k_csr_count"); k_csr_count<<<p.G, kFillThreads, 0, st>>>(p); }
    }
    const int vgrid = persistent_grid((long long)ls->Vcap, kThreads, 4);
    { LCCRF_KERNEL(ctx, "k_csr_prefix"); k_csr_prefix<<<vgrid, kThreads, 0, st>>>(p, b.B); }
    const int sgrid = persistent_grid((long long)ls->Vcap + 1, 1024, 2);
    { LCCRF_KERNEL(ctx, "k_scan_local"); k_scan_local<<<sgrid, 1024, 0, st>>>(ls->row_ptr, vt, ls->scan_tot); }
    { LCCRF_KERNEL(ctx, "k_scan_tot"); k_scan_tot<<<1, 1024, 0, st>>>(ls->scan_tot, vt); }
    { LCCRF_KERNEL(ctx, "k_scan_add"); k_scan_add<<<sgrid, 1024, 0, st>>>(ls->row_ptr, vt, ls->scan_tot); }
    if (p.G > 0) {
        LCCRF_TRY(ensure_dyn_smem(ctx, k_csr_fill, kCursorSmemInts * (int)sizeof(int)));
        { LCCRF_KERNEL(ctx, "k_csr_fill"); k_csr_fill<<<p.G, kFillWarpsH * 32, kCursorSmemInts * sizeof(int), st>>>(p); }
    }
    LCCRF_CUDA(cudaMemsetAsync(ls->row_counts, 0, 8 * sizeof(int), st));
    { LCCRF_KERNEL(ctx, "k_row_classify"); k_row_classify<<<vgrid, kThreads, 0, st>>>(ls->row_ptr, vt, ls->row_list_long, ls->row_counts, ls->piece_list); }
    if (ls->max_long > 0) {
        LCCRF_KERNEL(ctx, "k_long_chunks");
        k_long_chunks<<<1, 1024, 0, st>>>(ls->row_ptr, ls->row_list_long, ls->row_counts, ls->long_chunk0, (int4 *)ls->chunk_desc);
    }
    if (ls->n_tiles > 0) {
        LCCRF_CUDA(cudaMemsetAsync(ls->tile_own, 0, (size_t)ls->n_tiles * sizeof(int), st));
        LCCRF_KERNEL(ctx, "k_tile_rows");
        k_tile_rows<<<vgrid, kThreads, 0, st>>>(ls->row_ptr, vt, ls->tile_row0, ls->tile_own, ls->n_tiles);
    }
    LCCRF_CUDA(cudaGetLastError());
    return LCCRF_OK;
}

}
```

### lc-crf-slam_b200/csrc/engine.cuh

```cuda
#pragma once

#include <cstddef>
#include <functional>
#include <vector>

#include "common.cuh"

namespace lccrf {

struct Ctx;

struct LatticeSet {
    int d = 0, D = 0;
    float w = 0.f;
    float alpha = 0.f;
    int NT = 0, B = 0;
    int Vcap = 0;
    int *offset = nullptr;
    float *bary = nullptr;
    int2 *nbr = nullptr;
    int *vert_slot = nullptr;
    int *vert_prob = nullptr;
    int *vbase = nullptr;
    int *tab_base = nullptr;
    long long tab_slots = 0;
    float *norm = nullptr;
    int *row_ptr = nullptr;
    int2 *csr_ent = nullptr;
    int csr_chunks = 0;
    int *chunk_prob = nullptr, *chunk_s0 = nullptr, *chunk_s1 = nullptr, *prob_chunk0 = nullptr;
    long long *chunk_tbl = nullptr;
    int *csr_tbl = nullptr, *scan_tot = nullptr;
    int *row_list_long = nullptr;
    int *row_counts = nullptr;
    int *long_chunk0 = nullptr;
    void *chunk_desc = nullptr;
    unsigned long long *chunk_sum = nullptr;
    void *chunk_rec = nullptr;
    int max_long = 0, max_chunks = 0;
    int *piece_list = nullptr;
    int max_pieces = 0;
    int n_tiles = 0;
    int *tile_row0 = nullptr;
    int *tile_own = nullptr;
    int2 *tile_info = nullptr;
    float *tile_part = nullptr;
    float *valA = nullptr, *valB = nullptr;
    int Lmax = 0;
};

constexpr int kCsrChunkPoints = 4096;
constexpr int kLongRow = 1024;
constexpr int kScanChunk = 2048;
constexpr int kChunkRecBytes = 16 + 2 * 24 + 4 * (kScanChunk / 256) * 4;
constexpr int kTileGranule = 2048;
constexpr int kTreeTile = 2048;

struct Batch {
    Ctx *ctx = nullptr;
    int B = 0, NT = 0, L = 0;
    std::vector<int> h_prob_ptr;
    int *prob_ptr = nullptr;
    int maxN = 0;
    bool fused_blur = false;
    std::vector<LatticeSet *> lat;
    float *unary = nullptr, *cur = nullptr, *next = nullptr, *tmp = nullptr;
    short *map = nullptr;
};

struct Ctx {
    int device = 0;
    cudaStream_t stream = nullptr;
    bool own_stream = false;
    cudaStream_t copy_stream = nullptr;
    cudaStream_t d2h_stream = nullptr;
    uint64_t launches = 0;
    uint64_t scratch_gen = 0;
    int opt_graphs = 1;
    int opt_fused = 1;
    int opt_ordered_splat = 1;
    int opt_trace = 0;
    int opt_bulk_blur = 1;
    int opt_map_slack = 0;
    int opt_profile = 0;
    struct ProfRec {
        const char *name;
        cudaEvent_t a, b;
    };
    std::vector<ProfRec> prof;
    struct Scratch {
        void *p = nullptr;
        size_t bytes = 0;
    };
    struct BuildScratch {
        Scratch hash_keys[3], hash_first, hash_id, ent_slot, ids_status;
        bool hash_dirty = false;
    };
    BuildScratch bs[2];
    Scratch misc, feat, pinned_in, pinned_out, dev_io;
    cudaStream_t aux_stream = nullptr;
    cudaEvent_t ev_fork = nullptr, ev_join = nullptr;
    int opt_concurrent = 1;
    int branch = 0;
    cudaStream_t sub_stream[2] = {nullptr, nullptr};
    cudaEvent_t ev_sub_fork[2] = {nullptr, nullptr}, ev_sub_join[2] = {nullptr, nullptr};
    int opt_split_splat = 1;
    std::vector<const void *> smem_attr_done;
    int *d_status = nullptr;
    int *h_status = nullptr;
};

int ctx_scratch(Ctx *ctx, Ctx::Scratch &s, size_t bytes, bool pinned = false);

constexpr int kFusedBlurMaxN = 32768;
int batch_init(Ctx *ctx, Batch &b, int B, const int *prob_ptr, int L, bool with_state);
void batch_release(Ctx *ctx, Batch &b);
int check_status(Ctx *ctx);
int decode_status(int st);

struct GraphReplay {
    cudaGraphExec_t exec = nullptr;
    int same_shape_runs = 0;
    uint64_t launches = 0;
    uint64_t gen = 0;
};
void graph_drop(GraphReplay &g);
bool graph_will_capture(const Ctx *ctx, const GraphReplay &g);
int graph_run(Ctx *ctx, GraphReplay &g, const std::function<int()> &enqueue);

struct KernelScope {
    Ctx *c;
    int idx = -1;
    KernelScope(Ctx *ctx, const char *name) : c(ctx) {
        c->launches++;
        if (c->opt_profile) {
            Ctx::ProfRec r;
            r.name = name;
            if (cudaEventCreate(&r.a) == cudaSuccess && cudaEventCreate(&r.b) == cudaSuccess) {
                cudaEventRecord(r.a, c->stream);
                c->prof.push_back(r);
                idx = (int)c->prof.size() - 1;
            }
        }
    }
    ~KernelScope() {
        if (idx >= 0) cudaEventRecord(c->prof[idx].b, c->stream);
    }
};
#define LCCRF_KERNEL(ctx, name) ::lccrf::KernelScope _kscope_##__LINE__(ctx, name)
bool ctx_concurrent(const Ctx *ctx);
int ctx_fork(Ctx *ctx);
int ctx_join(Ctx *ctx);
struct AuxScope {
    Ctx *c;
    cudaStream_t saved;
    bool on;
    explicit AuxScope(Ctx *ctx, bool enable = true) : c(ctx), saved(ctx->stream), on(enable && ctx_concurrent(ctx)) {
        if (on) {
            c->stream = c->aux_stream;
            c->branch = 1;
        }
    }
    ~AuxScope() {
        if (on) {
            c->stream = saved;
            c->branch = 0;
        }
    }
};
template <typename Kernel>
inline int ensure_dyn_smem(Ctx *ctx, Kernel *kernel, int bytes) {
    const void *key = (const void *)kernel;
    for (const void *k : ctx->smem_attr_done)
        if (k == key) return LCCRF_OK;
    LCCRF_CUDA(cudaFuncSetAttribute(kernel, cudaFuncAttributeMaxDynamicSharedMemorySize, bytes));
    ctx->smem_attr_done.push_back(key);
    return LCCRF_OK;
}

int dev_alloc(Ctx *ctx, void **p, size_t bytes, bool zero = false);
void dev_free(Ctx *ctx, void *p);

struct KfPack {
    float4 r0, r1, r2, intr, bnd;
};

struct MapHeader {
    const KfPack *kf_packed;
    const float *pt_xyz;
    const int *pt_start, *pt_cnt;
    const int *pool_kf;
    const float *pool_uv;
    int n_kf;
};

struct DevMap {
    Ctx *ctx = nullptr;
    MapHeader *d_hdr = nullptr;
    cudaStream_t mstream = nullptr;
    cudaEvent_t ev_touch = nullptr, ev_mut = nullptr;
    int kp_stride = 0;
    int kf_cap = 0, n_kf = 0;
    KfPack *kf_packed = nullptr;
    float *kp_tab = nullptr;
    bool cam_set = false, ucam = true;
    float cam8[8] = {0, 0, 0, 0, 0, 0, 0, 0};
    int pt_cap = 0, n_pt = 0;
    float *pt_xyz = nullptr;
    int *pt_start = nullptr, *pt_cnt = nullptr, *pt_room = nullptr, *pt_stamp = nullptr;
    long long pool_cap = 0;
    int *pool_kf = nullptr;
    float *pool_uv = nullptr;
    int *d_ctr = nullptr;
    int *h_ctr = nullptr;
    cudaEvent_t ctr_ev = nullptr;
    bool ctr_pending = false;
    long long tail_seen = 0;
    long long tail_unseen = 0;
    int epoch = 0;
};

struct DeltaDev {
    int kf_first = 0, kf_count = 0;
    const float *kf_pose = nullptr, *kf_intr = nullptr, *kf_bounds = nullptr, *kf_keypoints = nullptr;
    int n_pose = 0;
    const int *pose_kf = nullptr;
    const float *pose = nullptr;
    int n_xyz = 0;
    const int *xyz_id = nullptr;
    const float *xyz = nullptr;
    int n_erase = 0;
    const int *erase_pt = nullptr, *erase_kf = nullptr;
    int n_bad = 0;
    const int *bad_pt = nullptr;
    int n_add = 0;
    const int *add_pt = nullptr, *add_kf = nullptr, *add_fid = nullptr;
    std::vector<int> erase_seg, add_seg;
};
size_t delta_stage_bytes(const lccrf_map_delta &d, int kp_stride, bool with_keypoints);
int delta_stage(const lccrf_map_delta &d, int kp_stride, bool with_keypoints, char *base, cudaStream_t st, DeltaDev *out);
int delta_grow_points(DevMap *m, const lccrf_map_delta &d);

int map_create(Ctx *ctx, int kp_stride, DevMap **out);
void map_destroy(DevMap *m);
int map_prepare(DevMap *m, const lccrf_map_delta &h);
int map_apply_dev(DevMap *m, const DeltaDev &d, const float *kp_host);
int map_bulk_observations(DevMap *m, int pt_first, int count, const int *obs_ptr_dev, const int *obs_ref_dev, long long nnz,
                          int slack_percent);
int map_publish(DevMap *m);
int map_begin_main_access(DevMap *m);
int map_end_main_access(DevMap *m);
int map_begin_async_mut(DevMap *m);
int map_end_async_mut(DevMap *m);
struct MapStreamScope {
    Ctx *c;
    cudaStream_t saved;
    explicit MapStreamScope(DevMap *m, bool enable = true) : c(m->ctx), saved(m->ctx->stream) {
        if (enable) c->stream = m->mstream;
    }
    ~MapStreamScope() { c->stream = saved; }
};
int map_reserve_pool(DevMap *m, long long entries);
int map_reserve_points(DevMap *m, int n);
int map_bulk_reserve(DevMap *m, long long need);
int map_export_dev(DevMap *m, int n, const int *ids_dev, int *cnt_dev);
int map_export_entries_dev(DevMap *m, int n, const int *ids_dev, const int *ptr_dev, int *kf_dev, float *uv_dev, float *xyz_dev,
                           long long cap);
int map_counters(DevMap *m, long long *tail, long long *live);

int lattice_set_create(Ctx *ctx, const Batch &b, int d, float w, int Lmax, LatticeSet **out);
void lattice_set_destroy(Ctx *ctx, LatticeSet *ls);
int lattice_set_build(Ctx *ctx, const Batch &b, LatticeSet *ls, const float *feat_dev);
int lattice_set_ensure_L(Ctx *ctx, LatticeSet *ls, int L);
int build_scratch_in_use(Ctx *ctx, long long *slots);
int csr_create(Ctx *ctx, const Batch &b, LatticeSet *ls);
void csr_destroy(Ctx *ctx, LatticeSet *ls);
int csr_build(Ctx *ctx, const Batch &b, LatticeSet *ls);
int filter_splat_blur(Ctx *ctx, const Batch &b, LatticeSet *ls, const float *in_dev, int L,
                      const float **values_out);
int filter_full(Ctx *ctx, const Batch &b, LatticeSet *ls, float *out_dev, const float *in_dev, int L);
int potts_norm(Ctx *ctx, const Batch &b, LatticeSet *ls);
int mf_unary_from_label(Ctx *ctx, float *unary, const short *label_dev, int NT, int L, float u_energy,
                        const float *n_en, const float *p_en, int *status = nullptr);
int mf_exp_and_normalize(Ctx *ctx, float *out, const float *in, int NT, int L, float scale, float relax);
int mf_start(Ctx *ctx, Batch &b);
int mf_step(Ctx *ctx, Batch &b, float relax);
int mf_build_map(Ctx *ctx, Batch &b);
int mf_negate(Ctx *ctx, float *out, const float *in, long long n);
int mf_potts_apply(Ctx *ctx, const Batch &b, LatticeSet *ls, float *out, const float *in, float *tmp, int L);
int mf_apply_fused(Ctx *ctx, const Batch &b, LatticeSet *ls, const float *cur, float *next, const float *unary,
                   bool first);
int launch_axpy_norm(Ctx *ctx, float *out, const float *tmp, const float *norm, float w, int NT, int L);
int mf_point_pass_l2(Ctx *ctx, Batch &b, const float *const *values, float relax, bool with_map);
int feat_div2(Ctx *ctx, float *feat, const float *a, int stride_a, float sa, const float *b, int stride_b,
              float sb, int N);
int feat_image(Ctx *ctx, float *feat, int W, int H, int F, float posdev, const void *img_dev, int is_u8,
               float featuredev);
int feat_image_batch(Ctx *ctx, float *feat, int NT, int B, const int *prob_ptr, const int *width, int F, float posdev,
                     const void *img_dev, int is_u8, float featuredev);
int unary_pack_kf(Ctx *ctx, void *kf_packed , const float *pose, const float *intr, const float *bnd, int nKF);
int unary_map_points_packed(Ctx *ctx, int N, int nKF, const float *xyz, const int *obs_ptr, const void *obs_kf,
                            int obs_kf_bytes, const float *obs_uv, const void *kf_packed, float *observs, float *error, float *depth,
                            const int *prob_ptr, const int *kf_ptr, int B, int kf_slice_max, const float *cam8,
                            const float *kp_tab, int kp_stride);
int unary_map_points_visible(Ctx *ctx, int N, const int *vis, const MapHeader *map_hdr, int n_kf_bucket, float *observs,
                             float *error, float *depth, const int *prob_ptr, const int *kf_ptr, int B, int kf_slice_max,
                             const float *cam8);
int unary_map_points(Ctx *ctx, int N, const float *xyz, const int *obs_ptr, const int *obs_kf,
                     const float *obs_uv, int nKF, const float *kf_pose, const float *kf_intr,
                     const float *kf_bounds, float *observs, float *error, float *depth, const float *cam8);
bool uniform_camera(const float *kf_intr, const float *kf_bounds, int nKF, float *cam8);
int unary_classify(Ctx *ctx, int N, const float *observs, const float *error, const float *depth,
                   const double *p4, const lccrf_slam_params &prm, short *label, const unsigned char *has_prior = nullptr,
                   const int *prob_ptr = nullptr, int B = 0);

size_t label_partition_scratch_bytes(int NT);
int label_partition(Ctx *ctx, const short *map, int NT, const int *prob_ptr, int B, const int *fid, int *scratch,
                    int *dyn_ptr, int *dyn_list, int *stat_ptr, int *stat_list);

int epipolar_prior(Ctx *ctx, int M, const int *fid1, const float *pt1, const float *pt2, const double *F9_host,
                   float u_gamma, float stdev_gamma, int nFeat, double *dis_by_fid, double *prob_by_fid, double *dis_m,
                   double *prob_m);
int bf_match_splits(int B, int max_nq, int max_nt);
int bf_match(Ctx *ctx, int B, int NQ, int max_nq, int max_nt, const int *q_ptr, const void *desc_q, const int *t_ptr,
             const void *desc_t, double ratio, int S, void *part , int *match, int *knn ,
             int *n_match);

}

struct lccrf_ctx {
    lccrf::Ctx c;
};

struct lccrf_map {
    lccrf::DevMap *m = nullptr;
};
```

### lc-crf-slam_b200/csrc/lattice_build.cu

```cuda
#include <climits>
#include <cmath>
#include <cstring>

#include "engine.cuh"

namespace lccrf {

namespace {

constexpr uint64_t kTag = 1ull << 63;

__host__ __device__ constexpr int num_levels(int d) { return d <= 3 ? 1 : 1 + (d - 3 + 1) / 2; }

struct BuildParams {
    int NT, B;
    const int *prob_ptr;
    const int *tab_base;
    const float *feat;
    uint64_t *key[3];
    int *first;
    int *tab_id;
    int *ent_slot;
    float *bary;
    int *offset;
    int2 *nbr;
    int *vert_slot, *vert_prob, *vbase;
    int Vcap;
    int *status;
    float scale[LCCRF_MAX_D];
    float invD, fD;
};

__device__ __forceinline__ int hash_insert(uint64_t *keys, int base, uint32_t mask, uint64_t word) {
    uint32_t h = mix64(word) & mask;
    for (;;) {
        uint64_t prev = __ldcg((const unsigned long long *)keys + base + h);
        if (prev == word) return base + (int)h;
        if (prev == 0ull) {
            prev = atomicCAS((unsigned long long *)keys + base + h, 0ull, (unsigned long long)word);
            if (prev == 0ull || prev == word) return base + (int)h;
        }
        h = (h + 1) & mask;
    }
}

__device__ __forceinline__ int hash_find(const uint64_t *keys, int base, uint32_t mask, uint64_t word) {
    uint32_t h = mix64(word) & mask;
    for (;;) {
        uint64_t k = __ldg((const unsigned long long *)keys + base + h);
        if (k == word) return base + (int)h;
        if (k == 0ull) return -1;
        h = (h + 1) & mask;
    }
}

template <int d>
__device__ __forceinline__ uint64_t word_level(const int *kc, int lev, int prev_local_slot) {
    if (lev == 0) {
        uint64_t w = kTag | (uint64_t)(uint16_t)kc[0];
        if (d > 1) w |= (uint64_t)(uint16_t)kc[1] << 16;
        if (d > 2) w |= (uint64_t)(uint16_t)kc[2] << 32;
        return w;
    }
    int c0 = 3 + 2 * (lev - 1);
    uint64_t w = kTag | ((uint64_t)(uint32_t)prev_local_slot << 32) | (uint64_t)(uint16_t)kc[c0];
    if (c0 + 1 < d) w |= (uint64_t)(uint16_t)kc[c0 + 1] << 16;
    return w;
}

__device__ __forceinline__ int pseudo_problem(const int *__restrict__ prob_ptr, int B, int ip) {
    int lo = 0, hi = B;
    while (hi - lo > 1) {
        int mid = (lo + hi) >> 1;
        if (__ldg(prob_ptr + mid) + mid <= ip) lo = mid;
        else hi = mid;
    }
    return lo;
}

template <int d>
__global__ void __launch_bounds__(kThreads) k_embed(BuildParams p) {
    constexpr int D = d + 1;
    constexpr int NLEV = num_levels(d);
    const int ip = blockIdx.x * kThreads + threadIdx.x;
    if (ip >= p.NT + p.B) return;
    const int b = pseudo_problem(p.prob_ptr, p.B, ip);
    const int p0 = __ldg(p.prob_ptr + b), p1 = __ldg(p.prob_ptr + b + 1);
    const int Nb = p1 - p0;
    const int local = ip - (p0 + b);
    const bool phantom = (local == Nb);
    int *es = p.ent_slot + (size_t)ip * D;
    if (phantom && (Nb & 3) == 0) {
#pragma unroll
        for (int r = 0; r < D; r++) es[r] = -1;
        return;
    }
    const int i = p0 + local;
    float f[d];
#pragma unroll
    for (int j = 0; j < d; j++) f[j] = phantom ? 0.0f : __ldg(p.feat + (size_t)i * d + j);

    float el[D];
    float sm = 0.0f;
#pragma unroll
    for (int j = d; j > 0; j--) {
        float cf = __fmul_rn(f[j - 1], p.scale[j - 1]);
        el[j] = __fsub_rn(sm, __fmul_rn((float)j, cf));
        sm = __fadd_rn(sm, cf);
    }
    el[0] = sm;
    float rem[D];
    int rank[D];
    int sum = 0;
#pragma unroll
    for (int q = 0; q < D; q++) {
        float v = rintf(__fmul_rn(p.invD, el[q]));
        rem[q] = __fmul_rn(v, p.fD);
        sum += (int)v;
        rank[q] = 0;
    }
#pragma unroll
    for (int a = 0; a < d; a++) {
        float da = __fsub_rn(el[a], rem[a]);
#pragma unroll
        for (int c = a + 1; c < D; c++) {
            float dc = __fsub_rn(el[c], rem[c]);
            if (da < dc) rank[a]++;
            else rank[c]++;
        }
    }
#pragma unroll
    for (int q = 0; q < D; q++) {
        rank[q] += sum;
        if (rank[q] < 0) {
            rank[q] += D;
            rem[q] = __fadd_rn(rem[q], p.fD);
        } else if (rank[q] >= D) {
            rank[q] -= D;
            rem[q] = __fsub_rn(rem[q], p.fD);
        }
    }
    float bc[D + 1];
#pragma unroll
    for (int q = 0; q <= D; q++) bc[q] = 0.0f;
#pragma unroll
    for (int a = 0; a < D; a++) {
        float v = __fmul_rn(__fsub_rn(el[a], rem[a]), p.invD);
        int pi = d - rank[a];
#pragma unroll
        for (int q = 0; q <= D; q++) {
            if (q == pi) bc[q] = __fadd_rn(bc[q], v);
            if (q == pi + 1) bc[q] = __fsub_rn(bc[q], v);
        }
    }
    bc[0] = __fadd_rn(bc[0], __fadd_rn(1.0f, bc[D]));

    const int base = __ldg(p.tab_base + b);
    const uint32_t mask = (uint32_t)(__ldg(p.tab_base + b + 1) - base) - 1u;
    bool range_ok = true;
#pragma unroll
    for (int r = 0; r < D; r++) {
        int kc[d];
#pragma unroll
        for (int c = 0; c < d; c++) {
            kc[c] = (int)rem[c] + ((rank[c] <= d - r) ? r : r - D);
            range_ok = range_ok && (kc[c] >= -32768 && kc[c] <= 32767);
        }
        int slot = 0;
#pragma unroll
        for (int lev = 0; lev < NLEV; lev++) {
            uint64_t w = word_level<d>(kc, lev, slot - base);
            slot = hash_insert(p.key[lev], base, mask, w);
        }
        if (__ldcg(p.first + slot) > ip * D + r) atomicMin(p.first + slot, ip * D + r);
        es[r] = slot;
        if (!phantom) p.bary[(size_t)i * D + r] = bc[r];
    }
    if (!range_ok) atomicOr(p.status, 1);
}

__device__ __forceinline__ bool is_first(const BuildParams &p, int s, int S, int &slot) {
    slot = -1;
    if (s >= S) return false;
    slot = __ldg(p.ent_slot + s);
    return slot >= 0 && __ldg(p.first + slot) == s;
}

constexpr int kIdThreads = 1024;
constexpr int kIdItems = 4;
constexpr int kIdTile = kIdThreads * kIdItems;
constexpr unsigned long long kIdCount = 1ull << 32, kIdPrefix = 2ull << 32;

__device__ __forceinline__ void id_publish(unsigned long long *p, unsigned long long w) {
    asm volatile("st.relaxed.gpu.global.u64 [%0], %1;" ::"l"(p), "l"(w) : "memory");
}
__device__ __forceinline__ unsigned long long id_poll(const unsigned long long *p) {
    unsigned long long w;
    asm volatile("ld.relaxed.gpu.global.u64 %0, [%1];" : "=l"(w) : "l"(p) : "memory");
    return w;
}

template <int D>
__global__ void __launch_bounds__(kIdThreads) k_vertex_ids(BuildParams p, unsigned long long *ids_status, int ntiles) {
    __shared__ int s_excl[kIdItems * 32];
    __shared__ unsigned s_bal[kIdItems * 32];
    __shared__ int s_tile, s_prefix, s_total;
    if (threadIdx.x == 0) s_tile = (int)atomicAdd(ids_status + ntiles, 1ull);
    __syncthreads();
    const int tile = s_tile;
    const int S = (p.NT + p.B) * D;
    const int s0 = tile * kIdTile;
    const int lane = threadIdx.x & 31, wid = threadIdx.x >> 5;
    int slot[kIdItems];
    unsigned bal[kIdItems];
#pragma unroll
    for (int j = 0; j < kIdItems; j++) {
        const bool f = is_first(p, s0 + j * kIdThreads + threadIdx.x, S, slot[j]);
        bal[j] = __ballot_sync(0xffffffffu, f);
        if (!f) slot[j] = -1;
        if (lane == 0) s_bal[j * 32 + wid] = bal[j];
    }
    __syncthreads();
    if (wid == 0) {
        int c[kIdItems], sum = 0;
#pragma unroll
        for (int k = 0; k < kIdItems; k++) {
            c[k] = __popc(s_bal[lane * kIdItems + k]);
            sum += c[k];
        }
        int incl = sum;
#pragma unroll
        for (int o = 1; o < 32; o <<= 1) {
            const int y = __shfl_up_sync(0xffffffffu, incl, o);
            if (lane >= o) incl += y;
        }
        int run = incl - sum;
#pragma unroll
        for (int k = 0; k < kIdItems; k++) {
            s_excl[lane * kIdItems + k] = run;
            run += c[k];
        }
        const int total = __shfl_sync(0xffffffffu, incl, 31);
        int prefix = 0;
        if (tile > 0) {
            if (lane == 0) id_publish(ids_status + tile, kIdCount | (unsigned)total);
            for (int pred = tile - 1;;) {
                const int t = pred - lane;
                const unsigned long long w = t >= 0 ? id_poll(ids_status + t) : kIdPrefix;
                if (__any_sync(0xffffffffu, (w >> 32) == 0)) continue;
                const unsigned pm = __ballot_sync(0xffffffffu, (w >> 32) == 2);
                const int stop = pm ? __ffs(pm) - 1 : 31;
                int v = lane <= stop ? (int)(unsigned)w : 0;
#pragma unroll
                for (int o = 16; o; o >>= 1) v += __shfl_xor_sync(0xffffffffu, v, o);
                prefix += v;
                if (pm) break;
                pred -= 32;
            }
        }
        if (lane == 0) {
            id_publish(ids_status + tile, kIdPrefix | (unsigned)(prefix + total));
            s_prefix = prefix;
            s_total = total;
        }
    }
    __syncthreads();
    const int prefix = s_prefix;
#pragma unroll
    for (int j = 0; j < kIdItems; j++) {
        if (slot[j] >= 0) {
            const int s = s0 + j * kIdThreads + threadIdx.x;
            const int id = prefix + s_excl[j * 32 + wid] + __popc(bal[j] & ((1u << lane) - 1u));
            p.tab_id[slot[j]] = id;
            p.vert_slot[id] = slot[j];
            p.vert_prob[id] = pseudo_problem(p.prob_ptr, p.B, s / D);
        }
    }
    const int s1 = s0 + kIdTile;
    const int b0 = s0 < S ? pseudo_problem(p.prob_ptr, p.B, s0 / D) : p.B;
    for (int b = b0 + (int)threadIdx.x; b < p.B; b += kIdThreads) {
        const int sb = (__ldg(p.prob_ptr + b) + b) * D;
        if (sb >= s1) break;
        if (sb >= s0) {
            const int q = sb - s0, g = q >> 5;
            p.vbase[b] = prefix + s_excl[g] + __popc(s_bal[g] & ((1u << (q & 31)) - 1u));
        }
    }
    if (tile == ntiles - 1 && threadIdx.x == 0) p.vbase[p.B] = prefix + s_total;
}

template <int D>
__global__ void __launch_bounds__(kThreads) k_offsets(BuildParams p) {
    const int i = blockIdx.x * kThreads + threadIdx.x;
    if (i >= p.NT) return;
    const int b = find_segment(p.prob_ptr, p.B + 1, i);
    const int *es = p.ent_slot + (size_t)(i + b) * D;
#pragma unroll
    for (int r = 0; r < D; r++) p.offset[(size_t)i * D + r] = __ldg(p.tab_id + __ldg(es + r));
}

template <int d>
__global__ void __launch_bounds__(kThreads) k_neighbours(BuildParams p) {
    constexpr int D = d + 1;
    constexpr int NLEV = num_levels(d);
    const int V = __ldg(p.vbase + p.B);
    const long long total = (long long)V * D;
    for (long long t = (long long)blockIdx.x * kThreads + threadIdx.x; t < total;
         t += (long long)gridDim.x * kThreads) {
        const int j = (int)(t / V), id = (int)(t - (long long)j * V);
        const int b = __ldg(p.vert_prob + id);
        const int base = __ldg(p.tab_base + b);
        const uint32_t mask = (uint32_t)(__ldg(p.tab_base + b + 1) - base) - 1u;
        int kc[d];
        int slot = __ldg(p.vert_slot + id);
#pragma unroll
        for (int lev = NLEV - 1; lev >= 0; lev--) {
            uint64_t w = __ldg((const unsigned long long *)p.key[lev] + slot);
            if (lev == 0) {
                kc[0] = (short)(w & 0xffff);
                if (d > 1) kc[1] = (short)((w >> 16) & 0xffff);
                if (d > 2) kc[2] = (short)((w >> 32) & 0xffff);
            } else {
                int c0 = 3 + 2 * (lev - 1);
                kc[c0] = (short)(w & 0xffff);
                if (c0 + 1 < d) kc[c0 + 1] = (short)((w >> 16) & 0xffff);
                slot = base + (int)((w >> 32) & 0x7fffffffu);
            }
        }
        int res[2];
#pragma unroll
        for (int side = 0; side < 2; side++) {
            int nk[d];
#pragma unroll
            for (int c = 0; c < d; c++) {
                int v = side == 0 ? kc[c] - 1 : kc[c] + 1;
                if (c == j) v = side == 0 ? kc[c] + d : kc[c] - d;
                nk[c] = (int)(short)v;
            }
            int sl = base;
            bool found = true;
#pragma unroll
            for (int lev = 0; lev < NLEV; lev++) {
                if (found) {
                    uint64_t w = word_level<d>(nk, lev, sl - base);
                    sl = hash_find(p.key[lev], base, mask, w);
                    found = sl >= 0;
                }
            }
            res[side] = found ? __ldg(p.tab_id + sl) : -1;
        }
        p.nbr[(size_t)j * p.Vcap + id] = make_int2(res[0], res[1]);
    }
}

template <int d>
__global__ void __launch_bounds__(kThreads) k_hash_clear(BuildParams p) {
    constexpr int NLEV = num_levels(d);
    const int V = __ldg(p.vbase + p.B);
    for (int id = blockIdx.x * kThreads + threadIdx.x; id < V; id += gridDim.x * kThreads) {
        int slot = __ldg(p.vert_slot + id);
        p.first[slot] = 0x7f7f7f7f;
        if (NLEV == 1) {
            p.key[0][slot] = 0ull;
            continue;
        }
        const int base = __ldg(p.tab_base + __ldg(p.vert_prob + id));
        uint64_t w = p.key[NLEV - 1][slot];
        p.key[NLEV - 1][slot] = 0ull;
#pragma unroll
        for (int lev = NLEV - 2; lev >= 0 && w != 0ull; lev--) {
            slot = base + (int)((w >> 32) & 0x7fffffffu);
            w = atomicExch((unsigned long long *)p.key[lev] + slot, 0ull);
        }
    }
}

template <int d>
int launch_build(Ctx *ctx, const BuildParams &p, unsigned long long *ids_status) {
    constexpr int D = d + 1;
    cudaStream_t st = ctx->stream;
    const int NP = p.NT + p.B;
    const long long S = (long long)NP * D;
    const int ntiles = S > 0 ? cdiv(S, kIdTile) : 1;
    const int vgrid = persistent_grid((long long)p.Vcap, kThreads, 4);
    { LCCRF_KERNEL(ctx, "k_embed"); k_embed<d><<<cdiv(NP, kThreads), kThreads, 0, st>>>(p); }
    LCCRF_CUDA(cudaMemsetAsync(ids_status, 0, ((size_t)ntiles + 1) * sizeof(unsigned long long), st));
    { LCCRF_KERNEL(ctx, "k_vertex_ids"); k_vertex_ids<D><<<ntiles, kIdThreads, 0, st>>>(p, ids_status, ntiles); }
    if (p.NT > 0) {
        { LCCRF_KERNEL(ctx, "k_offsets"); k_offsets<D><<<cdiv(p.NT, kThreads), kThreads, 0, st>>>(p); }
    }
    { LCCRF_KERNEL(ctx, "k_neighbours"); k_neighbours<d><<<vgrid, kThreads, 0, st>>>(p); }
    { LCCRF_KERNEL(ctx, "k_hash_clear"); k_hash_clear<d><<<vgrid, kThreads, 0, st>>>(p); }
    LCCRF_CUDA(cudaGetLastError());
    return LCCRF_OK;
}

}

int lattice_set_create(Ctx *ctx, const Batch &b, int d, float w, int Lmax, LatticeSet **out) {
    if (d < 1 || d > LCCRF_MAX_D) return fail(LCCRF_ERR_ARG, "feature dimension must be in [1, LCCRF_MAX_D]");
    auto *ls = new LatticeSet();
    ls->d = d;
    ls->D = d + 1;
    ls->w = w;
    ls->alpha = 1.0f / (1 + powf(2, (float)-d));
    ls->NT = b.NT;
    ls->B = b.B;
    ls->Lmax = Lmax;
    const long long vcap = ((long long)b.NT + b.B) * ls->D;
    if (vcap > INT_MAX / 2) {
        delete ls;
        return fail(LCCRF_ERR_ARG, "batch too large: (NT + B) * (d+1) must stay below 2^30");
    }
    ls->Vcap = (int)((vcap + 1) & ~1LL);
    const size_t nent = (size_t)(b.NT > 0 ? b.NT : 1) * ls->D;
    int rc = LCCRF_OK;
    rc |= dev_alloc(ctx, (void **)&ls->offset, nent * sizeof(int));
    rc |= dev_alloc(ctx, (void **)&ls->bary, nent * sizeof(float));
    rc |= dev_alloc(ctx, (void **)&ls->nbr, (size_t)ls->D * ls->Vcap * sizeof(int2));
    rc |= dev_alloc(ctx, (void **)&ls->vert_slot, (size_t)ls->Vcap * sizeof(int));
    rc |= dev_alloc(ctx, (void **)&ls->vert_prob, (size_t)ls->Vcap * sizeof(int));
    rc |= dev_alloc(ctx, (void **)&ls->vbase, (size_t)(b.B + 1) * sizeof(int));
    rc |= dev_alloc(ctx, (void **)&ls->norm, (size_t)(b.NT > 0 ? b.NT : 1) * sizeof(float));
    if (Lmax > 0) {
        rc |= dev_alloc(ctx, (void **)&ls->valA, (size_t)ls->Vcap * Lmax * sizeof(float));
        rc |= dev_alloc(ctx, (void **)&ls->valB, (size_t)ls->Vcap * Lmax * sizeof(float));
    }
    rc |= dev_alloc(ctx, (void **)&ls->tab_base, (size_t)(b.B + 1) * sizeof(int));
    {
        const long long E = (long long)b.NT * ls->D;
        const size_t mc = (size_t)(E / kScanChunk + E / kLongRow) + 1;
        if (Lmax > 0) {
            rc |= dev_alloc(ctx, (void **)&ls->chunk_sum, mc * Lmax * sizeof(unsigned long long), true);
            rc |= dev_alloc(ctx, (void **)&ls->chunk_rec, mc * Lmax * kChunkRecBytes);
        }
    }
    if (rc != LCCRF_OK) {
        lattice_set_destroy(ctx, ls);
        return LCCRF_ERR_CUDA;
    }
    std::vector<int> tab_base(b.B + 1);
    long long slots = 0;
    for (int i = 0; i < b.B; i++) {
        tab_base[i] = (int)slots;
        long long nb = b.h_prob_ptr[i + 1] - b.h_prob_ptr[i];
        long long need = 2 * ((nb + 3) / 4 * 4) * ls->D;
        long long sz = 64;
        while (sz < need) sz <<= 1;
        slots += sz;
        if (slots > INT_MAX) {
            lattice_set_destroy(ctx, ls);
            return fail(LCCRF_ERR_ARG, "hash table would exceed 2^31 slots");
        }
    }
    tab_base[b.B] = (int)slots;
    ls->tab_slots = slots;
    cudaError_t e = cudaMemcpyAsync(ls->tab_base, tab_base.data(), (size_t)(b.B + 1) * sizeof(int),
                                    cudaMemcpyHostToDevice, ctx->stream);
    if (e == cudaSuccess) e = cudaStreamSynchronize(ctx->stream);
    if (e != cudaSuccess) {
        lattice_set_destroy(ctx, ls);
        return fail(LCCRF_ERR_CUDA, std::string("tab_base upload: ") + cudaGetErrorString(e));
    }
    if (csr_create(ctx, b, ls) != LCCRF_OK) {
        lattice_set_destroy(ctx, ls);
        return LCCRF_ERR_CUDA;
    }
    *out = ls;
    return LCCRF_OK;
}

int lattice_set_ensure_L(Ctx *ctx, LatticeSet *ls, int L) {
    if (L <= ls->Lmax) return LCCRF_OK;
    if (L > LCCRF_MAX_L) return fail(LCCRF_ERR_ARG, "label count exceeds LCCRF_MAX_L");
    dev_free(ctx, ls->valA);
    dev_free(ctx, ls->valB);
    dev_free(ctx, ls->chunk_sum);
    dev_free(ctx, ls->chunk_rec);
    dev_free(ctx, ls->tile_part);
    ls->valA = ls->valB = nullptr;
    ls->chunk_sum = nullptr;
    ls->chunk_rec = nullptr;
    ls->tile_part = nullptr;
    ls->Lmax = 0;
    int rc = LCCRF_OK;
    {
        const size_t mc = (size_t)ls->max_chunks + 1;
        rc |= dev_alloc(ctx, (void **)&ls->chunk_sum, mc * L * sizeof(unsigned long long), true);
        rc |= dev_alloc(ctx, (void **)&ls->chunk_rec, mc * L * kChunkRecBytes);
    }
    rc |= dev_alloc(ctx, (void **)&ls->valA, (size_t)ls->Vcap * L * sizeof(float));
    rc |= dev_alloc(ctx, (void **)&ls->valB, (size_t)ls->Vcap * L * sizeof(float));
    rc |= dev_alloc(ctx, (void **)&ls->tile_part, ((size_t)ls->n_tiles + 1) * L * sizeof(float));
    if (rc != LCCRF_OK) return LCCRF_ERR_CUDA;
    ls->Lmax = L;
    return LCCRF_OK;
}

void lattice_set_destroy(Ctx *ctx, LatticeSet *ls) {
    if (!ls) return;
    dev_free(ctx, ls->offset);
    dev_free(ctx, ls->bary);
    dev_free(ctx, ls->nbr);
    dev_free(ctx, ls->vert_slot);
    dev_free(ctx, ls->vert_prob);
    dev_free(ctx, ls->vbase);
    dev_free(ctx, ls->norm);
    dev_free(ctx, ls->valA);
    dev_free(ctx, ls->valB);
    dev_free(ctx, ls->tab_base);
    csr_destroy(ctx, ls);
    delete ls;
}

namespace {

int build_enqueue(Ctx *ctx, const Batch &b, LatticeSet *ls, const float *feat_dev, Ctx::BuildScratch &bs, bool dirty) {
    const int d = ls->d, D = ls->D;
    const long long slots = ls->tab_slots;
    const int NLEV = num_levels(d);
    auto hash_region = [&](Ctx::Scratch &s, size_t bytes, int fill) -> int {
        const size_t had = s.p ? s.bytes : 0;
        LCCRF_TRY(ctx_scratch(ctx, s, bytes));
        if (s.bytes != had || dirty) LCCRF_CUDA(cudaMemsetAsync(s.p, fill, s.bytes, ctx->stream));
        return LCCRF_OK;
    };
    for (int lev = 0; lev < NLEV; lev++) LCCRF_TRY(hash_region(bs.hash_keys[lev], (size_t)slots * sizeof(uint64_t), 0));
    LCCRF_TRY(hash_region(bs.hash_first, (size_t)slots * sizeof(int), 0x7f));
    if (dirty) {
        for (int lev = NLEV; lev < 3; lev++)
            if (bs.hash_keys[lev].p) LCCRF_CUDA(cudaMemsetAsync(bs.hash_keys[lev].p, 0, bs.hash_keys[lev].bytes, ctx->stream));
    }
    LCCRF_TRY(ctx_scratch(ctx, bs.hash_id, (size_t)slots * sizeof(int)));
    const long long S = ((long long)b.NT + b.B) * D;
    LCCRF_TRY(ctx_scratch(ctx, bs.ent_slot, (size_t)S * sizeof(int)));
    const long long ntiles = S > 0 ? cdiv(S, kIdTile) : 1;
    LCCRF_TRY(ctx_scratch(ctx, bs.ids_status, (size_t)(ntiles + 1) * sizeof(unsigned long long)));

    BuildParams p;
    memset(&p, 0, sizeof(p));
    p.NT = b.NT;
    p.B = b.B;
    p.prob_ptr = b.prob_ptr;
    p.tab_base = ls->tab_base;
    p.feat = feat_dev;
    for (int lev = 0; lev < NLEV; lev++) p.key[lev] = (uint64_t *)bs.hash_keys[lev].p;
    p.first = (int *)bs.hash_first.p;
    p.tab_id = (int *)bs.hash_id.p;
    p.ent_slot = (int *)bs.ent_slot.p;
    p.bary = ls->bary;
    p.offset = ls->offset;
    p.nbr = ls->nbr;
    p.vert_slot = ls->vert_slot;
    p.vert_prob = ls->vert_prob;
    p.vbase = ls->vbase;
    p.Vcap = ls->Vcap;
    p.status = ctx->d_status;
    float inv_std_dev = (float)(sqrt(2.0 / 3.0) * (d + 1));
    for (int i = 0; i < d; i++) p.scale[i] = (float)(1.0 / sqrt((double)((i + 2) * (i + 1))) * (double)inv_std_dev);
    p.invD = 1.0f / (d + 1);
    p.fD = (float)(d + 1);
    unsigned long long *ids_status = (unsigned long long *)bs.ids_status.p;
    int rc = LCCRF_ERR_ARG;
    switch (d) {
        case 1: rc = launch_build<1>(ctx, p, ids_status); break;
        case 2: rc = launch_build<2>(ctx, p, ids_status); break;
        case 3: rc = launch_build<3>(ctx, p, ids_status); break;
        case 4: rc = launch_build<4>(ctx, p, ids_status); break;
        case 5: rc = launch_build<5>(ctx, p, ids_status); break;
        case 6: rc = launch_build<6>(ctx, p, ids_status); break;
        case 7: rc = launch_build<7>(ctx, p, ids_status); break;
        default: return fail(LCCRF_ERR_ARG, "unsupported feature dimension");
    }
    return rc;
}

}

__global__ void k_hash_in_use(const uint64_t *key, const int *first, long long n, unsigned long long *count) {
    unsigned long long c = 0;
    for (long long i = (long long)blockIdx.x * kThreads + threadIdx.x; i < n; i += (long long)gridDim.x * kThreads)
        c += (key && key[i] != 0ull) || (first && first[i] != 0x7f7f7f7f);
    if (c) atomicAdd(count, c);
}

int build_scratch_in_use(Ctx *ctx, long long *slots) {
    unsigned long long *d_count = nullptr, h_count = 0;
    LCCRF_CUDA(cudaStreamSynchronize(ctx->stream));
    if (ctx->aux_stream) LCCRF_CUDA(cudaStreamSynchronize(ctx->aux_stream));
    LCCRF_CUDA(cudaMalloc(&d_count, sizeof(unsigned long long)));
    cudaError_t e = cudaMemset(d_count, 0, sizeof(unsigned long long));
    for (const Ctx::BuildScratch &bs : ctx->bs) {
        for (const Ctx::Scratch &k : bs.hash_keys)
            if (e == cudaSuccess && k.p) {
                k_hash_in_use<<<persistent_grid((long long)(k.bytes / 8), kThreads, 4), kThreads>>>((const uint64_t *)k.p, nullptr, (long long)(k.bytes / 8), d_count);
                e = cudaGetLastError();
            }
        if (e == cudaSuccess && bs.hash_first.p) {
            k_hash_in_use<<<persistent_grid((long long)(bs.hash_first.bytes / 4), kThreads, 4), kThreads>>>(nullptr, (const int *)bs.hash_first.p, (long long)(bs.hash_first.bytes / 4), d_count);
            e = cudaGetLastError();
        }
    }
    if (e == cudaSuccess) e = cudaMemcpy(&h_count, d_count, sizeof(h_count), cudaMemcpyDeviceToHost);
    cudaFree(d_count);
    if (e != cudaSuccess) return fail(LCCRF_ERR_CUDA, std::string("build_scratch_in_use: ") + cudaGetErrorString(e));
    *slots = (long long)h_count;
    return LCCRF_OK;
}

int lattice_set_build(Ctx *ctx, const Batch &b, LatticeSet *ls, const float *feat_dev) {
    Ctx::BuildScratch &bs = ctx->bs[ctx->branch];
    const bool dirty = bs.hash_dirty;
    bs.hash_dirty = true;
    const int rc = build_enqueue(ctx, b, ls, feat_dev, bs, dirty);
    if (rc != LCCRF_OK) {
        ctx->scratch_gen++;
        return rc;
    }
    bs.hash_dirty = false;
    return csr_build(ctx, b, ls);
}

}
```

Baseline: 8635.

## Fuse CSR offset computation, row scan and classification; sort-based CSR fill

The per-entry offset kernel is folded into the CSR count kernel, which now counts in shared memory when a problem's vertex count fits. The zero, prefix, three-pass scan, row classification and tile-row kernels are replaced by one persistent kernel that uses a decoupled look-back scan, now shared with the vertex-id kernel. The CSR fill is rewritten to radix-sort each tile of entries in shared memory before scattering. The aim is fewer launches and fewer global passes in lattice construction, at the cost of more complex code, spin-wait dependencies between tiles, and larger shared-memory use. A CSR export API is also added.

```diff
diff --git a/include/lccrf.h b/include/lccrf.h
--- a/include/lccrf.h
+++ b/include/lccrf.h
@@ -38,6 +38,7 @@
 void lccrf_lattice_destroy(lccrf_lattice *lat);
 int lccrf_lattice_sizes(const lccrf_lattice *lat, int *N, int *d, int *V);
 int lccrf_lattice_export(const lccrf_lattice *lat, int *offset, float *bary, int *nbr);
+int lccrf_lattice_export_csr(const lccrf_lattice *lat, int *row_ptr, int *entries);
 int lccrf_lattice_filter(lccrf_lattice *lat, float *out, const float *in, int L);
 int lccrf_lattice_filter_window(lccrf_lattice *lat, float *out, const float *in, int L, int in_offset, int out_offset,
                                 int in_size, int out_size);
diff --git a/lc-crf-slam_b200/__init__.py b/lc-crf-slam_b200/__init__.py
--- a/lc-crf-slam_b200/__init__.py
+++ b/lc-crf-slam_b200/__init__.py
@@ -66,6 +66,7 @@
     "lccrf_lattice_destroy": (None, [_vp]),
     "lccrf_lattice_sizes": (C.c_int, [_vp, _ip, _ip, _ip]),
     "lccrf_lattice_export": (C.c_int, [_vp, _vp, _vp, _vp]),
+    "lccrf_lattice_export_csr": (C.c_int, [_vp, _vp, _vp]),
     "lccrf_lattice_filter": (C.c_int, [_vp, _vp, _vp, C.c_int]),
     "lccrf_lattice_filter_window": (C.c_int, [_vp, _vp, _vp, C.c_int, C.c_int, C.c_int, C.c_int, C.c_int]),
     "lccrf_crf_create": (C.c_int, [_vp, C.c_int, C.c_int, C.POINTER(_vp)]),
@@ -319,6 +320,12 @@
         self.ctx._check(self.ctx.lib.lccrf_lattice_export(self.h, _ptr(off), _ptr(bary), _ptr(nbr)))
         return off, bary, nbr
 
+    def export_csr(self):
+        row_ptr = np.empty(self.V + 1, dtype=np.int32)
+        ent = np.empty((self.N * (self.d + 1), 2), dtype=np.int32)
+        self.ctx._check(self.ctx.lib.lccrf_lattice_export_csr(self.h, _ptr(row_ptr), _ptr(ent)))
+        return row_ptr, ent
+
     def filter(self, x) -> np.ndarray:
         x = _arr(x, np.float32)
         L = x.size // self.N if self.N else 1
diff --git a/lc-crf-slam_b200/csrc/api.cu b/lc-crf-slam_b200/csrc/api.cu
--- a/lc-crf-slam_b200/csrc/api.cu
+++ b/lc-crf-slam_b200/csrc/api.cu
@@ -465,6 +465,18 @@
             LCCRF_CUDA(cudaMemcpyAsync(nbr + 2 * (size_t)j * lat->V, ls->nbr + (size_t)j * ls->Vcap,
                                        (size_t)lat->V * sizeof(int2), cudaMemcpyDeviceToHost, ctx->stream));
     }
+    LCCRF_CUDA(cudaStreamSynchronize(ctx->stream));
+    return LCCRF_OK;
+}
+
+int lccrf_lattice_export_csr(const lccrf_lattice *lat, int *row_ptr, int *entries) {
+    if (!lat) return fail(LCCRF_ERR_ARG, "lattice is NULL");
+    Ctx *ctx = lat->ctx;
+    LCCRF_CUDA(cudaSetDevice(ctx->device));
+    const LatticeSet *ls = lat->ls;
+    const size_t nent = (size_t)lat->b.NT * ls->D;
+    if (row_ptr) LCCRF_CUDA(cudaMemcpyAsync(row_ptr, ls->row_ptr, ((size_t)lat->V + 1) * sizeof(int), cudaMemcpyDeviceToHost, ctx->stream));
+    if (entries && nent) LCCRF_CUDA(cudaMemcpyAsync(entries, ls->csr_ent, nent * sizeof(int2), cudaMemcpyDeviceToHost, ctx->stream));
     LCCRF_CUDA(cudaStreamSynchronize(ctx->stream));
     return LCCRF_OK;
 }
diff --git a/lc-crf-slam_b200/csrc/common.cuh b/lc-crf-slam_b200/csrc/common.cuh
--- a/lc-crf-slam_b200/csrc/common.cuh
+++ b/lc-crf-slam_b200/csrc/common.cuh
@@ -47,6 +47,48 @@
     return (uint32_t)x;
 }
 
+constexpr unsigned long long kTileCount = 1ull << 32, kTilePrefix = 2ull << 32;
+
+__device__ __forceinline__ void tile_publish(unsigned long long *p, unsigned long long w) {
+    asm volatile("st.relaxed.gpu.global.u64 [%0], %1;" ::"l"(p), "l"(w) : "memory");
+}
+__device__ __forceinline__ unsigned long long tile_poll(const unsigned long long *p) {
+    unsigned long long w;
+    asm volatile("ld.relaxed.gpu.global.u64 %0, [%1];" : "=l"(w) : "l"(p) : "memory");
+    return w;
+}
+
+__device__ __forceinline__ int tile_lookback(unsigned long long *status, int tile, int total, unsigned payload,
+                                             unsigned *pred_payload) {
+    const int lane = threadIdx.x & 31;
+    const unsigned long long pay = (unsigned long long)payload << 34;
+    int prefix = 0;
+    unsigned pp = 0;
+    if (tile > 0) {
+        if (lane == 0) tile_publish(status + tile, pay | kTileCount | (unsigned)total);
+        bool first = true;
+        for (int pred = tile - 1;;) {
+            const int t = pred - lane;
+            const unsigned long long w = t >= 0 ? tile_poll(status + t) : kTilePrefix;
+            const unsigned f = (unsigned)(w >> 32) & 3u;
+            if (__any_sync(0xffffffffu, f == 0)) continue;
+            if (first) pp = __shfl_sync(0xffffffffu, (unsigned)(w >> 34), 0);
+            first = false;
+            const unsigned pm = __ballot_sync(0xffffffffu, f == 2);
+            const int stop = pm ? __ffs(pm) - 1 : 31;
+            int v = lane <= stop ? (int)(unsigned)w : 0;
+#pragma unroll
+            for (int o = 16; o; o >>= 1) v += __shfl_xor_sync(0xffffffffu, v, o);
+            prefix += v;
+            if (pm) break;
+            pred -= 32;
+        }
+    }
+    if (lane == 0) tile_publish(status + tile, pay | kTilePrefix | (unsigned)(prefix + total));
+    *pred_payload = pp;
+    return prefix;
+}
+
 __device__ __forceinline__ int find_segment(const int *__restrict__ arr, int n, int x) {
     int lo = 0, hi = n;
     while (hi - lo > 1) {
diff --git a/lc-crf-slam_b200/csrc/csr.cu b/lc-crf-slam_b200/csrc/csr.cu
--- a/lc-crf-slam_b200/csrc/csr.cu
+++ b/lc-crf-slam_b200/csrc/csr.cu
@@ -1,3 +1,5 @@
+#include <cub/block/block_radix_sort.cuh>
+
 #include "engine.cuh"
 
 namespace lccrf {
@@ -5,7 +7,7 @@
 namespace {
 
 constexpr int kFillThreads = 1024;
-constexpr int kCursorSmemInts = 14336;
+constexpr int kSharedV = 8192;
 
 struct CsrParams {
     int G;
@@ -15,7 +17,9 @@
     const int *chunk_s1;
     const long long *chunk_tbl;
     const int *prob_chunk0;
-    const int *offset;
+    const int *ent_slot;
+    const int *tab_id;
+    int *offset;
     const float *bary;
     const int *vbase;
     const int *vert_prob;
@@ -24,131 +28,158 @@
     int2 *ent;
 };
 
-__global__ void __launch_bounds__(kThreads) k_csr_zero(CsrParams p) {
-    const int g = blockIdx.x;
-    const int b = __ldg(p.chunk_prob + g);
-    const int Vb = __ldg(p.vbase + b + 1) - __ldg(p.vbase + b);
-    int *row = p.tbl + __ldg(p.chunk_tbl + g);
-    for (int v = threadIdx.x; v < Vb; v += kThreads) row[v] = 0;
-}
-
-__global__ void __launch_bounds__(kFillThreads) k_csr_count(CsrParams p) {
+
+__global__ void __launch_bounds__(kFillThreads) k_offsets(CsrParams p) {
+    __shared__ int s_cnt[kSharedV];
     const int g = blockIdx.x;
     const int b = __ldg(p.chunk_prob + g);
     const int vb = __ldg(p.vbase + b);
+    const int Vb = __ldg(p.vbase + b + 1) - vb;
     int *row = p.tbl + __ldg(p.chunk_tbl + g);
+    int *cnt = Vb <= kSharedV ? s_cnt : row;
     const int s0 = __ldg(p.chunk_s0 + g), s1 = __ldg(p.chunk_s1 + g);
+    const int *es = p.ent_slot + (size_t)b * p.D;
     const unsigned lane = threadIdx.x & 31;
+    for (int v = threadIdx.x; v < Vb; v += kFillThreads) cnt[v] = 0;
+    __syncthreads();
     for (int base = s0; base < s1; base += 4 * kFillThreads) {
         int v[4];
 #pragma unroll
         for (int j = 0; j < 4; j++) {
             const int s = base + j * kFillThreads + threadIdx.x;
-            v[j] = s < s1 ? __ldg(p.offset + s) - vb : -1;
+            v[j] = s < s1 ? __ldg(p.tab_id + __ldg(es + s)) : -1;
         }
 #pragma unroll
         for (int j = 0; j < 4; j++) {
-            const unsigned grp = __match_any_sync(0xffffffffu, v[j]);
-            if (v[j] >= 0 && (__ffs(grp) - 1) == (int)lane) atomicAdd(row + v[j], __popc(grp));
-        }
-    }
-}
-
-__global__ void __launch_bounds__(kThreads) k_csr_prefix(CsrParams p, int B) {
+            const int s = base + j * kFillThreads + threadIdx.x;
+            if (v[j] >= 0) p.offset[s] = v[j];
+            const int lv = v[j] >= 0 ? v[j] - vb : -1;
+            const unsigned grp = __match_any_sync(0xffffffffu, lv);
+            if (lv >= 0 && (__ffs(grp) - 1) == (int)lane) atomicAdd(cnt + lv, __popc(grp));
+        }
+    }
+    if (cnt == s_cnt) {
+        __syncthreads();
+        for (int v = threadIdx.x; v < Vb; v += kFillThreads) row[v] = s_cnt[v];
+    }
+}
+
+constexpr int kRowThreads = 1024;
+constexpr int kRowAhead = 8;
+
+struct RowOut {
+    int *row_ptr;
+    int *lng;
+    int *counts;
+    int *piece_list;
+    int *tile_row0;
+    int *tile_own;
+    int n_tiles;
+    unsigned long long *status;
+    int ntiles_cap;
+};
+
+__global__ void __launch_bounds__(kRowThreads) k_csr_rows(CsrParams p, int B, RowOut o) {
+    __shared__ int ws[32];
+    __shared__ int s_len[kRowThreads];
+    __shared__ int s_tile, s_prefix, s_prev_len;
     const int V = __ldg(p.vbase + B);
-    for (int v = blockIdx.x * kThreads + threadIdx.x; v < V; v += gridDim.x * kThreads) {
-        const int b = __ldg(p.vert_prob + v);
-        const int lv = v - __ldg(p.vbase + b);
-        const int g0 = __ldg(p.prob_chunk0 + b), g1 = __ldg(p.prob_chunk0 + b + 1);
-        int run = 0;
-        for (int g = g0; g < g1; g++) {
-            int *c = p.tbl + __ldg(p.chunk_tbl + g) + lv;
-            const int n = *c;
-            *c = run;
-            run += n;
-        }
-        p.row_len[v] = run;
-    }
-}
-
-__global__ void __launch_bounds__(1024) k_scan_local(int *x, const int *n_ptr, int *blk_tot) {
-    __shared__ int ws[32];
-    const int n = __ldg(n_ptr);
-    const int lane = threadIdx.x & 31, wid = threadIdx.x >> 5;
-    for (int blk = blockIdx.x; blk * 1024 < n + 1; blk += gridDim.x) {
-        const int idx = blk * 1024 + threadIdx.x;
-        const int v = idx < n ? x[idx] : 0;
-        int s = v;
-#pragma unroll
-        for (int o = 1; o < 32; o <<= 1) {
-            int y = __shfl_up_sync(0xffffffffu, s, o);
-            if (lane >= o) s += y;
-        }
-        if (lane == 31) ws[wid] = s;
+    const int ntiles = V / kRowThreads + 1;
+    const int tid = threadIdx.x, lane = tid & 31, wid = tid >> 5;
+    for (;;) {
+        if (tid == 0) s_tile = (int)atomicAdd(o.status + o.ntiles_cap, 1ull);
+        __syncthreads();
+        const int tile = s_tile;
+        if (tile >= ntiles) break;
+        const int v = tile * kRowThreads + tid;
+        int len = 0;
+        if (v < V) {
+            const int b = __ldg(p.vert_prob + v);
+            const int lv = v - __ldg(p.vbase + b);
+            const int g0 = __ldg(p.prob_chunk0 + b), g1 = __ldg(p.prob_chunk0 + b + 1);
+            for (int g = g0; g < g1; g += kRowAhead) {
+                int *c[kRowAhead];
+                int n[kRowAhead];
+#pragma unroll
+                for (int k = 0; k < kRowAhead; k++) {
+                    c[k] = g + k < g1 ? p.tbl + __ldg(p.chunk_tbl + g + k) + lv : nullptr;
+                    n[k] = c[k] ? *c[k] : 0;
+                }
+#pragma unroll
+                for (int k = 0; k < kRowAhead; k++) {
+                    if (c[k]) *c[k] = len;
+                    len += n[k];
+                }
+            }
+        }
+        s_len[tid] = len;
+        int incl = len;
+#pragma unroll
+        for (int off = 1; off < 32; off <<= 1) {
+            const int y = __shfl_up_sync(0xffffffffu, incl, off);
+            if (lane >= off) incl += y;
+        }
+        if (lane == 31) ws[wid] = incl;
         __syncthreads();
         if (wid == 0) {
             int t = ws[lane];
 #pragma unroll
-            for (int o = 1; o < 32; o <<= 1) {
-                int y = __shfl_up_sync(0xffffffffu, t, o);
-                if (lane >= o) t += y;
+            for (int off = 1; off < 32; off <<= 1) {
+                const int y = __shfl_up_sync(0xffffffffu, t, off);
+                if (lane >= off) t += y;
             }
             ws[lane] = t;
-        }
-        __syncthreads();
-        const int excl = (wid ? ws[wid - 1] : 0) + s - v;
-        if (idx <= n) x[idx] = excl;
-        if (threadIdx.x == 1023) blk_tot[blk] = ws[31];
-        __syncthreads();
-    }
-}
-
-__global__ void __launch_bounds__(1024) k_scan_tot(int *blk_tot, const int *n_ptr) {
-    __shared__ int ws[32];
-    __shared__ int carry_s;
-    const int nblk = (__ldg(n_ptr) + 1 + 1023) / 1024;
-    if (threadIdx.x == 0) carry_s = 0;
-    __syncthreads();
-    const int lane = threadIdx.x & 31, wid = threadIdx.x >> 5;
-    for (int start = 0; start < nblk; start += 1024) {
-        const int idx = start + threadIdx.x;
-        const int v = idx < nblk ? blk_tot[idx] : 0;
-        int s = v;
-#pragma unroll
-        for (int o = 1; o < 32; o <<= 1) {
-            int y = __shfl_up_sync(0xffffffffu, s, o);
-            if (lane >= o) s += y;
-        }
-        if (lane == 31) ws[wid] = s;
-        __syncthreads();
-        if (wid == 0) {
-            int t = ws[lane];
-#pragma unroll
-            for (int o = 1; o < 32; o <<= 1) {
-                int y = __shfl_up_sync(0xffffffffu, t, o);
-                if (lane >= o) t += y;
-            }
-            ws[lane] = t;
-        }
-        __syncthreads();
-        const int carry = carry_s;
-        if (idx < nblk) blk_tot[idx] = carry + (wid ? ws[wid - 1] : 0) + s - v;
-        __syncthreads();
-        if (threadIdx.x == 1023) carry_s = carry + ws[31];
-        __syncthreads();
-    }
-}
-
-__global__ void __launch_bounds__(1024) k_scan_add(int *x, const int *n_ptr, const int *blk_tot) {
-    const int n = __ldg(n_ptr);
-    for (int blk = blockIdx.x; blk * 1024 < n + 1; blk += gridDim.x) {
-        const int idx = blk * 1024 + threadIdx.x;
-        if (idx <= n) x[idx] += __ldg(blk_tot + blk);
-    }
-}
-
-constexpr int kFillWarpsH = 8;
-constexpr int kHierV = kCursorSmemInts / kFillWarpsH;
+            const int total = __shfl_sync(0xffffffffu, t, 31);
+            unsigned prev_len;
+            const int prefix = tile_lookback(o.status, tile, total, (unsigned)s_len[kRowThreads - 1], &prev_len);
+            if (lane == 0) {
+                s_prefix = prefix;
+                s_prev_len = (int)prev_len;
+            }
+        }
+        __syncthreads();
+        const int start = s_prefix + (wid ? ws[wid - 1] : 0) + incl - len;
+        if (v <= V) o.row_ptr[v] = start;
+        if (v < V) {
+            if (len >= kLongRow) {
+                o.lng[atomicAdd(o.counts, 1)] = v;
+            } else {
+                bool first = v == 0;
+                if (!first) {
+                    const int plen = tid ? s_len[tid - 1] : s_prev_len;
+                    first = plen >= kLongRow || start / kTileGranule != (start - plen) / kTileGranule;
+                }
+                if (first) o.piece_list[atomicAdd(o.counts + 2, 1)] = v;
+            }
+            const int e = start + len;
+            for (int t = (start + kTreeTile - 1) / kTreeTile; t < o.n_tiles && t * kTreeTile < e; t++) o.tile_row0[t] = v;
+            if (len < kLongRow && o.n_tiles > 0) {
+                const int t = e > start ? start / kTreeTile : (start > 0 ? (start - 1) / kTreeTile : 0);
+                o.tile_own[t < o.n_tiles ? t : o.n_tiles - 1] = 1;
+            }
+        }
+        if (v == V && o.n_tiles > 0) o.tile_row0[o.n_tiles] = V - 1;
+        __syncthreads();
+    }
+}
+
+constexpr int kSortThreads = 512;
+constexpr int kSortItems = 8;
+constexpr int kSortTile = kSortThreads * kSortItems;
+constexpr int kSortIdxBits = 12;
+static_assert(kSortTile == 1 << kSortIdxBits, "tile index field");
+static_assert((long long)kSharedV << kSortIdxBits < (1ll << 31), "sort key");
+using TileSort = cub::BlockRadixSort<int, kSortThreads, kSortItems>;
+
+struct FillSmem {
+    union {
+        typename TileSort::TempStorage sort;
+        int key[kSortTile + kSortTile / 32];
+    } u;
+    float bary[kSortTile];
+    int cur[kSharedV];
+};
+constexpr int kWalkSmemInts = (int)(sizeof(FillSmem) / sizeof(int));
 
 constexpr int kFillAhead = 4;
 
@@ -190,8 +221,56 @@
     }
 }
 
-__global__ void __launch_bounds__(kFillWarpsH * 32) k_csr_fill(CsrParams p) {
-    extern __shared__ int s_cur[];
+__device__ __forceinline__ void fill_sorted(const CsrParams &p, int vb, int Vb, int s0, int s1, const int *row,
+                                            FillSmem &sm) {
+    const int t = threadIdx.x;
+    for (int v = t; v < Vb; v += kSortThreads) sm.cur[v] = __ldg(p.row_len + vb + v) + row[v];
+    const int end_bit = kSortIdxBits + 32 - __clz(Vb);
+    for (int base = s0; base < s1; base += kSortTile) {
+        const int n = min(kSortTile, s1 - base);
+#pragma unroll
+        for (int k = 0; k < kSortItems; k++) {
+            const int i = k * kSortThreads + t;
+            sm.u.key[i + (i >> 5)] = ((i < n ? __ldg(p.offset + base + i) - vb : Vb) << kSortIdxBits) | i;
+            sm.bary[i] = i < n ? __ldg(p.bary + base + i) : 0.f;
+        }
+        __syncthreads();
+        int keys[kSortItems];
+#pragma unroll
+        for (int k = 0; k < kSortItems; k++) {
+            const int i = t * kSortItems + k;
+            keys[k] = sm.u.key[i + (i >> 5)];
+        }
+        __syncthreads();
+        TileSort(sm.u.sort).SortBlockedToStriped(keys, kSortIdxBits, end_bit);
+        __syncthreads();
+#pragma unroll
+        for (int k = 0; k < kSortItems; k++) sm.u.key[k * kSortThreads + t] = keys[k] >> kSortIdxBits;
+        __syncthreads();
+#pragma unroll
+        for (int k = 0; k < kSortItems; k++) {
+            const int j = k * kSortThreads + t, v = keys[k] >> kSortIdxBits;
+            if (j < n && (j == 0 || sm.u.key[j - 1] != v)) sm.cur[v] -= j;
+        }
+        __syncthreads();
+#pragma unroll
+        for (int k = 0; k < kSortItems; k++) {
+            const int j = k * kSortThreads + t, v = keys[k] >> kSortIdxBits, i = keys[k] & (kSortTile - 1);
+            if (j < n) p.ent[sm.cur[v] + j] = make_int2((base + i) / p.D, __float_as_int(sm.bary[i]));
+        }
+        __syncthreads();
+#pragma unroll
+        for (int k = 0; k < kSortItems; k++) {
+            const int j = k * kSortThreads + t, v = keys[k] >> kSortIdxBits;
+            if (j < n && (j == n - 1 || sm.u.key[j + 1] != v)) sm.cur[v] += j + 1;
+        }
+        __syncthreads();
+    }
+}
+
+__global__ void __launch_bounds__(kSortThreads, 2) k_csr_fill(CsrParams p) {
+    extern __shared__ __align__(16) unsigned char s_raw[];
+    FillSmem &sm = *reinterpret_cast<FillSmem *>(s_raw);
     const int g = blockIdx.x;
     const int b = __ldg(p.chunk_prob + g);
     const int vb = __ldg(p.vbase + b);
@@ -199,66 +278,16 @@
     int *row = p.tbl + __ldg(p.chunk_tbl + g);
     const int s0 = __ldg(p.chunk_s0 + g), s1 = __ldg(p.chunk_s1 + g);
     const unsigned lane = threadIdx.x & 31;
-    const int wid = threadIdx.x >> 5;
-    if (Vb <= kHierV) {
-        const int sub = ((s1 - s0 + kFillWarpsH - 1) / kFillWarpsH + 31) & ~31;
-        const int a = min(s0 + wid * sub, s1), z = min(a + sub, s1);
-        int *mine = s_cur + wid * Vb;
-        for (int v = threadIdx.x; v < kFillWarpsH * Vb; v += kFillWarpsH * 32) s_cur[v] = 0;
-        __syncthreads();
-        for (int base0 = a; base0 < z; base0 += 32 * kFillAhead) {
-            int vv[kFillAhead];
-#pragma unroll
-            for (int g = 0; g < kFillAhead; g++) {
-                const int s = base0 + 32 * g + (int)lane;
-                vv[g] = s < z ? __ldg(p.offset + s) - vb : -1;
-            }
-#pragma unroll
-            for (int g = 0; g < kFillAhead; g++) {
-                const unsigned grp = __match_any_sync(0xffffffffu, vv[g]);
-                if (vv[g] >= 0 && (__ffs(grp) - 1) == (int)lane) mine[vv[g]] += __popc(grp);
-                __syncwarp();
-            }
-        }
-        __syncthreads();
-        for (int v = threadIdx.x; v < Vb; v += kFillWarpsH * 32) {
-            int run = row[v];
-#pragma unroll
-            for (int w = 0; w < kFillWarpsH; w++) {
-                const int n = s_cur[w * Vb + v];
-                s_cur[w * Vb + v] = run;
-                run += n;
-            }
-        }
-        __syncthreads();
-        fill_walk<0>(p, vb, a, z, mine, lane);
-    } else if (wid == 0) {
-        if (Vb <= kCursorSmemInts) {
+    if (Vb <= kSharedV) {
+        fill_sorted(p, vb, Vb, s0, s1, row, sm);
+    } else if (threadIdx.x < 32) {
+        int *s_cur = reinterpret_cast<int *>(s_raw);
+        if (Vb <= kWalkSmemInts) {
             for (int v = (int)lane; v < Vb; v += 32) s_cur[v] = row[v];
             __syncwarp();
             fill_walk<1>(p, vb, s0, s1, s_cur, lane);
         } else {
             fill_walk<2>(p, vb, s0, s1, row, lane);
-        }
-    }
-}
-
-__global__ void __launch_bounds__(kThreads)
-k_row_classify(const int *__restrict__ row_ptr, const int *__restrict__ vtotal, int *__restrict__ lng,
-               int *__restrict__ counts, int *__restrict__ piece_list) {
-    const int V = __ldg(vtotal);
-    for (int v = blockIdx.x * kThreads + threadIdx.x; v < V; v += gridDim.x * kThreads) {
-        const int start = __ldg(row_ptr + v);
-        const int len = __ldg(row_ptr + v + 1) - start;
-        if (len >= kLongRow) {
-            lng[atomicAdd(counts, 1)] = v;
-        } else {
-            bool first = v == 0;
-            if (!first) {
-                const int pstart = __ldg(row_ptr + v - 1);
-                first = (start - pstart >= kLongRow) || (start / kTileGranule != pstart / kTileGranule);
-            }
-            if (first) piece_list[atomicAdd(counts + 2, 1)] = v;
         }
     }
 }
@@ -313,21 +342,6 @@
     if (threadIdx.x == 0) {
         long_chunk0[n] = carry_s;
         counts[1] = carry_s;
-    }
-}
-
-__global__ void __launch_bounds__(kThreads)
-k_tile_rows(const int *__restrict__ row_ptr, const int *__restrict__ vtotal, int *__restrict__ tile_row0,
-            int *__restrict__ tile_own, int n_tiles) {
-    const int V = __ldg(vtotal);
-    if (blockIdx.x == 0 && threadIdx.x == 0) tile_row0[n_tiles] = V - 1;
-    for (int v = blockIdx.x * kThreads + threadIdx.x; v < V; v += gridDim.x * kThreads) {
-        const int s = __ldg(row_ptr + v), e = __ldg(row_ptr + v + 1);
-        for (int t = (s + kTreeTile - 1) / kTreeTile; t < n_tiles && t * kTreeTile < e; t++) tile_row0[t] = v;
-        if (e - s < kLongRow && n_tiles > 0) {
-            const int t = e > s ? s / kTreeTile : (s > 0 ? (s - 1) / kTreeTile : 0);
-            tile_own[t < n_tiles ? t : n_tiles - 1] = 1;
-        }
     }
 }
 
@@ -373,7 +387,7 @@
     rc |= dev_alloc(ctx, (void **)&ls->csr_tbl, (size_t)(tbl > 0 ? tbl : 1) * 4);
     rc |= dev_alloc(ctx, (void **)&ls->row_ptr, ((size_t)ls->Vcap + 2) * 4);
     rc |= dev_alloc(ctx, (void **)&ls->csr_ent, (size_t)(b.NT > 0 ? b.NT : 1) * D * sizeof(int2));
-    rc |= dev_alloc(ctx, (void **)&ls->scan_tot, ((size_t)ls->Vcap / 1024 + 2) * 4);
+    rc |= dev_alloc(ctx, (void **)&ls->row_status, ((size_t)ls->Vcap / kRowThreads + 2) * sizeof(unsigned long long));
     {
         const long long E = (long long)b.NT * D;
         ls->max_long = (int)(E / kLongRow);
@@ -412,7 +426,7 @@
     dev_free(ctx, ls->csr_tbl);
     dev_free(ctx, ls->row_ptr);
     dev_free(ctx, ls->csr_ent);
-    dev_free(ctx, ls->scan_tot);
+    dev_free(ctx, ls->row_status);
     dev_free(ctx, ls->row_list_long);
     dev_free(ctx, ls->long_chunk0);
     dev_free(ctx, ls->chunk_desc);
@@ -426,7 +440,7 @@
     dev_free(ctx, ls->tile_part);
 }
 
-int csr_build(Ctx *ctx, const Batch &b, LatticeSet *ls) {
+int csr_build(Ctx *ctx, const Batch &b, LatticeSet *ls, const int *ent_slot, const int *tab_id) {
     cudaStream_t st = ctx->stream;
     CsrParams p;
     p.G = ls->csr_chunks;
@@ -436,6 +450,8 @@
     p.chunk_s1 = ls->chunk_s1;
     p.chunk_tbl = ls->chunk_tbl;
     p.prob_chunk0 = ls->prob_chunk0;
+    p.ent_slot = ent_slot;
+    p.tab_id = tab_id;
     p.offset = ls->offset;
     p.bary = ls->bary;
     p.vbase = ls->vbase;
@@ -443,32 +459,32 @@
     p.tbl = ls->csr_tbl;
     p.row_len = ls->row_ptr;
     p.ent = ls->csr_ent;
-    const int *vt = ls->vbase + ls->B;
+    if (p.G > 0) { LCCRF_KERNEL(ctx, "k_offsets"); k_offsets<<<p.G, kFillThreads, 0, st>>>(p); }
+    RowOut o;
+    o.row_ptr = ls->row_ptr;
+    o.lng = ls->row_list_long;
+    o.counts = ls->row_counts;
+    o.piece_list = ls->piece_list;
+    o.tile_row0 = ls->tile_row0;
+    o.tile_own = ls->tile_own;
+    o.n_tiles = ls->n_tiles;
+    o.status = ls->row_status;
+    o.ntiles_cap = ls->Vcap / kRowThreads + 1;
+    LCCRF_CUDA(cudaMemsetAsync(ls->row_status, 0, ((size_t)o.ntiles_cap + 1) * sizeof(unsigned long long), st));
+    LCCRF_CUDA(cudaMemsetAsync(ls->row_counts, 0, 8 * sizeof(int), st));
+    if (ls->n_tiles > 0) LCCRF_CUDA(cudaMemsetAsync(ls->tile_own, 0, (size_t)ls->n_tiles * sizeof(int), st));
+    {
+        LCCRF_KERNEL(ctx, "k_csr_rows");
+        k_csr_rows<<<persistent_grid((long long)ls->Vcap + 1, kRowThreads, 1), kRowThreads, 0, st>>>(p, b.B, o);
+    }
     if (p.G > 0) {
-        { LCCRF_KERNEL(ctx, "k_csr_zero"); k_csr_zero<<<p.G, kThreads, 0, st>>>(p); }
-        { LCCRF_KERNEL(ctx, "k_csr_count"); k_csr_count<<<p.G, kFillThreads, 0, st>>>(p); }
-    }
-    const int vgrid = persistent_grid((long long)ls->Vcap, kThreads, 4);
-    { LCCRF_KERNEL(ctx, "k_csr_prefix"); k_csr_prefix<<<vgrid, kThreads, 0, st>>>(p, b.B); }
-    const int sgrid = persistent_grid((long long)ls->Vcap + 1, 1024, 2);
-    { LCCRF_KERNEL(ctx, "k_scan_local"); k_scan_local<<<sgrid, 1024, 0, st>>>(ls->row_ptr, vt, ls->scan_tot); }
-    { LCCRF_KERNEL(ctx, "k_scan_tot"); k_scan_tot<<<1, 1024, 0, st>>>(ls->scan_tot, vt); }
-    { LCCRF_KERNEL(ctx, "k_scan_add"); k_scan_add<<<sgrid, 1024, 0, st>>>(ls->row_ptr, vt, ls->scan_tot); }
-    if (p.G > 0) {
-        LCCRF_TRY(ensure_dyn_smem(ctx, k_csr_fill, kCursorSmemInts * (int)sizeof(int)));
-        { LCCRF_KERNEL(ctx, "k_csr_fill"); k_csr_fill<<<p.G, kFillWarpsH * 32, kCursorSmemInts * sizeof(int), st>>>(p); }
-    }
-    LCCRF_CUDA(cudaMemsetAsync(ls->row_counts, 0, 8 * sizeof(int), st));
-    { LCCRF_KERNEL(ctx, "k_row_classify"); k_row_classify<<<vgrid, kThreads, 0, st>>>(ls->row_ptr, vt, ls->row_list_long, ls->row_counts, ls->piece_list); }
+        LCCRF_TRY(ensure_dyn_smem(ctx, k_csr_fill, (int)sizeof(FillSmem)));
+        { LCCRF_KERNEL(ctx, "k_csr_fill"); k_csr_fill<<<p.G, kSortThreads, sizeof(FillSmem), st>>>(p); }
+    }
     if (ls->max_long > 0) {
         LCCRF_KERNEL(ctx, "k_long_chunks");
         k_long_chunks<<<1, 1024, 0, st>>>(ls->row_ptr, ls->row_list_long, ls->row_counts, ls->long_chunk0, (int4 *)ls->chunk_desc);
     }
-    if (ls->n_tiles > 0) {
-        LCCRF_CUDA(cudaMemsetAsync(ls->tile_own, 0, (size_t)ls->n_tiles * sizeof(int), st));
-        LCCRF_KERNEL(ctx, "k_tile_rows");
-        k_tile_rows<<<vgrid, kThreads, 0, st>>>(ls->row_ptr, vt, ls->tile_row0, ls->tile_own, ls->n_tiles);
-    }
     LCCRF_CUDA(cudaGetLastError());
     return LCCRF_OK;
 }
diff --git a/lc-crf-slam_b200/csrc/engine.cuh b/lc-crf-slam_b200/csrc/engine.cuh
--- a/lc-crf-slam_b200/csrc/engine.cuh
+++ b/lc-crf-slam_b200/csrc/engine.cuh
@@ -30,7 +30,8 @@
     int csr_chunks = 0;
     int *chunk_prob = nullptr, *chunk_s0 = nullptr, *chunk_s1 = nullptr, *prob_chunk0 = nullptr;
     long long *chunk_tbl = nullptr;
-    int *csr_tbl = nullptr, *scan_tot = nullptr;
+    int *csr_tbl = nullptr;
+    unsigned long long *row_status = nullptr;
     int *row_list_long = nullptr;
     int *row_counts = nullptr;
     int *long_chunk0 = nullptr;
@@ -275,7 +276,7 @@
 int build_scratch_in_use(Ctx *ctx, long long *slots);
 int csr_create(Ctx *ctx, const Batch &b, LatticeSet *ls);
 void csr_destroy(Ctx *ctx, LatticeSet *ls);
-int csr_build(Ctx *ctx, const Batch &b, LatticeSet *ls);
+int csr_build(Ctx *ctx, const Batch &b, LatticeSet *ls, const int *ent_slot, const int *tab_id);
 int filter_splat_blur(Ctx *ctx, const Batch &b, LatticeSet *ls, const float *in_dev, int L,
                       const float **values_out);
 int filter_full(Ctx *ctx, const Batch &b, LatticeSet *ls, float *out_dev, const float *in_dev, int L);
diff --git a/lc-crf-slam_b200/csrc/lattice_build.cu b/lc-crf-slam_b200/csrc/lattice_build.cu
--- a/lc-crf-slam_b200/csrc/lattice_build.cu
+++ b/lc-crf-slam_b200/csrc/lattice_build.cu
@@ -189,16 +189,6 @@
 constexpr int kIdThreads = 1024;
 constexpr int kIdItems = 4;
 constexpr int kIdTile = kIdThreads * kIdItems;
-constexpr unsigned long long kIdCount = 1ull << 32, kIdPrefix = 2ull << 32;
-
-__device__ __forceinline__ void id_publish(unsigned long long *p, unsigned long long w) {
-    asm volatile("st.relaxed.gpu.global.u64 [%0], %1;" ::"l"(p), "l"(w) : "memory");
-}
-__device__ __forceinline__ unsigned long long id_poll(const unsigned long long *p) {
-    unsigned long long w;
-    asm volatile("ld.relaxed.gpu.global.u64 %0, [%1];" : "=l"(w) : "l"(p) : "memory");
-    return w;
-}
 
 template <int D>
 __global__ void __launch_bounds__(kIdThreads) k_vertex_ids(BuildParams p, unsigned long long *ids_status, int ntiles) {
@@ -241,25 +231,9 @@
             run += c[k];
         }
         const int total = __shfl_sync(0xffffffffu, incl, 31);
-        int prefix = 0;
-        if (tile > 0) {
-            if (lane == 0) id_publish(ids_status + tile, kIdCount | (unsigned)total);
-            for (int pred = tile - 1;;) {
-                const int t = pred - lane;
-                const unsigned long long w = t >= 0 ? id_poll(ids_status + t) : kIdPrefix;
-                if (__any_sync(0xffffffffu, (w >> 32) == 0)) continue;
-                const unsigned pm = __ballot_sync(0xffffffffu, (w >> 32) == 2);
-                const int stop = pm ? __ffs(pm) - 1 : 31;
-                int v = lane <= stop ? (int)(unsigned)w : 0;
-#pragma unroll
-                for (int o = 16; o; o >>= 1) v += __shfl_xor_sync(0xffffffffu, v, o);
-                prefix += v;
-                if (pm) break;
-                pred -= 32;
-            }
-        }
+        unsigned unused;
+        const int prefix = tile_lookback(ids_status, tile, total, 0u, &unused);
         if (lane == 0) {
-            id_publish(ids_status + tile, kIdPrefix | (unsigned)(prefix + total));
             s_prefix = prefix;
             s_total = total;
         }
@@ -287,16 +261,6 @@
         }
     }
     if (tile == ntiles - 1 && threadIdx.x == 0) p.vbase[p.B] = prefix + s_total;
-}
-
-template <int D>
-__global__ void __launch_bounds__(kThreads) k_offsets(BuildParams p) {
-    const int i = blockIdx.x * kThreads + threadIdx.x;
-    if (i >= p.NT) return;
-    const int b = find_segment(p.prob_ptr, p.B + 1, i);
-    const int *es = p.ent_slot + (size_t)(i + b) * D;
-#pragma unroll
-    for (int r = 0; r < D; r++) p.offset[(size_t)i * D + r] = __ldg(p.tab_id + __ldg(es + r));
 }
 
 template <int d>
@@ -386,9 +350,6 @@
     { LCCRF_KERNEL(ctx, "k_embed"); k_embed<d><<<cdiv(NP, kThreads), kThreads, 0, st>>>(p); }
     LCCRF_CUDA(cudaMemsetAsync(ids_status, 0, ((size_t)ntiles + 1) * sizeof(unsigned long long), st));
     { LCCRF_KERNEL(ctx, "k_vertex_ids"); k_vertex_ids<D><<<ntiles, kIdThreads, 0, st>>>(p, ids_status, ntiles); }
-    if (p.NT > 0) {
-        { LCCRF_KERNEL(ctx, "k_offsets"); k_offsets<D><<<cdiv(p.NT, kThreads), kThreads, 0, st>>>(p); }
-    }
     { LCCRF_KERNEL(ctx, "k_neighbours"); k_neighbours<d><<<vgrid, kThreads, 0, st>>>(p); }
     { LCCRF_KERNEL(ctx, "k_hash_clear"); k_hash_clear<d><<<vgrid, kThreads, 0, st>>>(p); }
     LCCRF_CUDA(cudaGetLastError());
@@ -618,7 +579,7 @@
         return rc;
     }
     bs.hash_dirty = false;
-    return csr_build(ctx, b, ls);
-}
-
-}
+    return csr_build(ctx, b, ls, (const int *)bs.ent_slot.p, (const int *)bs.hash_id.p);
+}
+
+}
```

New measurement: 9006, median of 6. 4.3% higher.
